# facebook/transform360

Measured on NVIDIA H100. Metric: Mpixels/s 8K equirect->cubemap bicubic (input-plane pixels consumed per second), higher is better.
Workload: dtype u8

## Files before the change

### include/transform360_b200.h

```cpp
#ifndef TRANSFORM360_B200_EXT_H
#define TRANSFORM360_B200_EXT_H

#include "Transform360/VideoFrameTransformHandler.h"

#ifdef __cplusplus
extern "C" {
#endif

typedef struct T360HostPlan T360HostPlan;

T360HostPlan* T360B200_hostPlanCreate(const FrameTransformContext* ctx, int inputWidth, int inputHeight,
                                      int outputWidth, int outputHeight);
#define T360_BORDER_WRAP 3
#define T360_BORDER_TRANSPARENT 5
T360HostPlan* T360B200_hostPlanCreateFromWarp(const FrameTransformContext* ctx, const float* map, int mapWidth, int mapHeight,
                                              int inputWidth, int inputHeight, int border);
void T360B200_hostPlanDestroy(T360HostPlan* plan);
int T360B200_hostPlanInfo(const T360HostPlan* plan, int info[6]);
const float* T360B200_hostPlanMap(const T360HostPlan* plan);
const int32_t* T360B200_hostPlanSamples(const T360HostPlan* plan);
int T360B200_hostPlanGather(T360HostPlan* plan, int info[10], const int32_t** jobs, const int32_t** records,
                            const uint32_t** compact);
int T360B200_hostPlanPoleCaps(T360HostPlan* plan, int info[4], const int32_t** capJobs, const uint32_t** capRecords,
                              const int32_t** launchJobs);
int T360B200_hostPlanDeviceLists(T360HostPlan* plan, int info[2], const int32_t** jobs, const uint32_t** records);
int T360B200_dealLanes(int interpolationAlg, int n, const int32_t* phases, int32_t* laneOf, int32_t* copyOf);
int T360B200_weightImage(int interpolationAlg, const uint8_t** image);
int T360B200_hostPlanBlurLists(T360HostPlan* const* plans, int numPlans, int width, int height, int layout[15],
                               const uint8_t** image);
int T360B200_hostPlanSegment(const T360HostPlan* plan, int i, int rect[4], int numTaps[2], const float** kx,
                             const float** ky);
int T360B200_remapTable(int interpolationAlg, const int16_t** table);

int T360B200_generateMapFromWarp(VideoFrameTransform* transform, const float* map, int mapWidth, int mapHeight, int inputWidth,
                                 int inputHeight, int border, int transformMatPlaneIndex);
int T360B200_remapFrameAsync(VideoFrameTransform* transform, int numPlanes, const float* const* deviceMaps, const int* mapPitches,
                             int border, const uint8_t* const* deviceInputs, uint8_t* const* deviceOutputs, const int* inputWidths,
                             const int* inputHeights, const int* inputPitches, const int* outputWidths, const int* outputHeights,
                             const int* outputPitches, void* cudaStream);

int T360B200_transformFramePlaneAsync(VideoFrameTransform* transform, const uint8_t* deviceInput,
                                      uint8_t* deviceOutput, int inputWidth, int inputHeight, int inputPitch,
                                      int outputWidth, int outputHeight, int outputPitch,
                                      int transformMatPlaneIndex, void* cudaStream);
int T360B200_transformFrameAsync(VideoFrameTransform* transform, int numPlanes, const uint8_t* const* deviceInputs,
                                 uint8_t* const* deviceOutputs, const int* inputWidths, const int* inputHeights,
                                 const int* inputPitches, const int* outputWidths, const int* outputHeights,
                                 const int* outputPitches, void* cudaStream);
int T360B200_lowPassPlaneAsync(VideoFrameTransform* transform, const uint8_t* deviceInput, uint8_t* deviceOutput,
                               int width, int height, int inputPitch, int outputPitch,
                               int transformMatPlaneIndex, void* cudaStream);
int T360B200_reconfigure(VideoFrameTransform* transform, const FrameTransformContext* ctx);
int T360B200_reconfigureAsync(VideoFrameTransform* transform, const FrameTransformContext* ctx);
int T360B200_reconfigureWait(VideoFrameTransform* transform, int block);
typedef struct T360View {
  float yaw, pitch, hfov, vfov;
} T360View;
int T360B200_transformFrameViewAsync(VideoFrameTransform* transform, const T360View* view, int numPlanes,
                                     const uint8_t* const* deviceInputs, uint8_t* const* deviceOutputs, const int* inputWidths,
                                     const int* inputHeights, const int* inputPitches, const int* outputWidths,
                                     const int* outputHeights, const int* outputPitches, void* cudaStream);
int T360B200_viewSamples(const FrameTransformContext* ctx, const T360View* view, int inputWidth, int inputHeight,
                         int outputWidth, int outputHeight, int32_t* samples);
typedef struct T360Orientation {
  float yaw, pitch, roll;
} T360Orientation;
int T360B200_transformFrameOrientedAsync(VideoFrameTransform* transform, const T360Orientation* orientation, int numPlanes,
                                         const uint8_t* const* deviceInputs, uint8_t* const* deviceOutputs,
                                         const int* inputWidths, const int* inputHeights, const int* inputPitches,
                                         const int* outputWidths, const int* outputHeights, const int* outputPitches,
                                         void* cudaStream);
int T360B200_orientedSamples(const FrameTransformContext* ctx, const T360Orientation* orientation, int inputWidth,
                             int inputHeight, int outputWidth, int outputHeight, int32_t* samples);
typedef struct T360Pose {
  float yaw, pitch, roll, hfov, vfov;
} T360Pose;
int T360B200_transformFramePoseAsync(VideoFrameTransform* transform, const T360Pose* pose, int numPlanes,
                                     const uint8_t* const* deviceInputs, uint8_t* const* deviceOutputs, const int* inputWidths,
                                     const int* inputHeights, const int* inputPitches, const int* outputWidths,
                                     const int* outputHeights, const int* outputPitches, void* cudaStream);
int T360B200_poseSamples(const FrameTransformContext* ctx, const T360Pose* pose, int inputWidth, int inputHeight,
                         int outputWidth, int outputHeight, int32_t* samples);
typedef struct T360Lens {
  float fx, fy, cx, cy;
  float k[4];
  float yaw, pitch, roll;
  float maxAngle;
} T360Lens;
typedef struct T360LensRig {
  int numLenses, calibWidth, calibHeight;
  T360Lens lens[2];
} T360LensRig;
int T360B200_lensMap(const FrameTransformContext* ctx, const T360LensRig* rig, const T360Orientation* orientation, int inputWidth,
                     int inputHeight, int outputWidth, int outputHeight, float* map);
int T360B200_transformFrameLensAsync(VideoFrameTransform* transform, const T360LensRig* rig, const T360Orientation* orientation,
                                     int numPlanes, const uint8_t* const* deviceInputs, uint8_t* const* deviceOutputs,
                                     const int* inputWidths, const int* inputHeights, const int* inputPitches,
                                     const int* outputWidths, const int* outputHeights, const int* outputPitches, void* cudaStream);
int T360B200_lensBlendMaps(const FrameTransformContext* ctx, const T360LensRig* rig, float seamWidth, const T360Orientation* orientation,
                           int inputWidth, int inputHeight, int outputWidth, int outputHeight, float* map0, float* map1, uint16_t* weight);
int T360B200_transformFrameLensBlendAsync(VideoFrameTransform* transform, const T360LensRig* rig, float seamWidth,
                                          const T360Orientation* orientation, int numPlanes, const uint8_t* const* deviceInputs,
                                          uint8_t* const* deviceOutputs, const int* inputWidths, const int* inputHeights,
                                          const int* inputPitches, const int* outputWidths, const int* outputHeights,
                                          const int* outputPitches, void* cudaStream);
int T360B200_rectilinearMap(const FrameTransformContext* ctx, const T360LensRig* rig, const T360Pose* pose, int inputWidth, int inputHeight,
                            int outputWidth, int outputHeight, float* map);
int T360B200_transformFrameRectilinearAsync(VideoFrameTransform* transform, const T360LensRig* rig, const T360Pose* pose, int numPlanes,
                                            const uint8_t* const* deviceInputs, uint8_t* const* deviceOutputs, const int* inputWidths,
                                            const int* inputHeights, const int* inputPitches, const int* outputWidths,
                                            const int* outputHeights, const int* outputPitches, void* cudaStream);
#define T360_CAMERA_PINHOLE 0
#define T360_CAMERA_EQUIDISTANT 1
#define T360_CAMERA_STEREOGRAPHIC 2
#define T360_CAMERA_PANNINI 3
typedef struct T360Camera {
  int model;
  float pannini;
} T360Camera;
int T360B200_cameraMap(const FrameTransformContext* ctx, const T360LensRig* rig, const T360Pose* pose, const T360Camera* camera,
                       int inputWidth, int inputHeight, int outputWidth, int outputHeight, float* map);
int T360B200_transformFrameCameraAsync(VideoFrameTransform* transform, const T360LensRig* rig, const T360Pose* pose, const T360Camera* camera,
                                       int numPlanes, const uint8_t* const* deviceInputs, uint8_t* const* deviceOutputs,
                                       const int* inputWidths, const int* inputHeights, const int* inputPitches, const int* outputWidths,
                                       const int* outputHeights, const int* outputPitches, void* cudaStream);
void T360B200_setPinHostPlanes(VideoFrameTransform* transform, int enable);
void T360B200_debugTrace(VideoFrameTransform* transform, int enable);
unsigned long long T360B200_debugTraceRead(VideoFrameTransform* transform, unsigned long long* out, unsigned long long maxWords);
int T360B200_synchronize(VideoFrameTransform* transform);
void* T360B200_stream(VideoFrameTransform* transform);

unsigned long long T360B200_kernelLaunchCount(void);
unsigned long long T360B200_planDeviceBytes(VideoFrameTransform* transform, int transformMatPlaneIndex);
int T360B200_planTileCounts(VideoFrameTransform* transform, int transformMatPlaneIndex, int counts[4]);
int T360B200_deviceCount(void);
const char* T360B200_version(void);

#ifdef __cplusplus
}
#endif
#endif
```

### transform360_b200/__init__.py

```python
from .handler import (BORDER_TRANSPARENT, BORDER_WRAP, CUBIC, LANCZOS4, LAYOUT_BARREL, LAYOUT_BARREL_SPLIT, LAYOUT_CUBEMAP_23_OFFCENTER,
                      LAYOUT_CUBEMAP_32, LAYOUT_EAC_32, LAYOUT_EQUIRECT, LAYOUT_FLAT_FIXED, LINEAR, NEAREST,
                      STEREO_FORMAT_GUESS, STEREO_FORMAT_LR, STEREO_FORMAT_MONO, STEREO_FORMAT_TB, T360_CAMERA_EQUIDISTANT, T360_CAMERA_PANNINI,
                      T360_CAMERA_PINHOLE, T360_CAMERA_STEREOGRAPHIC,
                      FrameTransformContext, HostPlan, T360Camera, T360Lens, T360LensRig, T360Orientation, T360Pose, T360View, VideoFrameTransform, device_count, kernel_launch_count,
                      camera_map, lens_blend_maps, lens_map, load, make_context, oriented_samples, pose_samples, rectilinear_map, remap_table,
                      square_pixel_vfov, view_samples, weight_image, deal_lanes)
```

### transform360_b200/csrc/gather_frame.cu

```cuda
#include "gather_common.cuh"

#include <cuda.h>

#include <algorithm>
#include <cstring>
#include <utility>

namespace t360 {

namespace {

template <class F, int... I>
__device__ __forceinline__ void staticForImpl(F&& f, std::integer_sequence<int, I...>) {
  (f(std::integral_constant<int, I>{}), ...);
}
template <int N, class F>
__device__ __forceinline__ void staticFor(F&& f) {
  staticForImpl(f, std::make_integer_sequence<int, N>{});
}

template <int IMM>
__device__ __forceinline__ uint32_t ldsWordImm(uint32_t addr) {
  uint32_t v;
  asm volatile("ld.shared.u32 %0, [%1+%2];" : "=r"(v) : "r"(addr), "n"(IMM));
  return v;
}
template <int IMM>
__device__ __forceinline__ uint4 ldsVecImm(uint32_t addr) {
  uint4 v;
  asm volatile("ld.shared.v4.u32 {%0, %1, %2, %3}, [%4+%5];" : "=r"(v.x), "=r"(v.y), "=r"(v.z), "=r"(v.w) : "r"(addr), "n"(IMM));
  return v;
}
template <int IMM>
__device__ __forceinline__ uint2 ldsVec2Imm(uint32_t addr) {
  uint2 v;
  asm volatile("ld.shared.v2.u32 {%0, %1}, [%2+%3];" : "=r"(v.x), "=r"(v.y) : "r"(addr), "n"(IMM));
  return v;
}

__device__ __forceinline__ uint32_t smemAddr(const void* p) { return (uint32_t)__cvta_generic_to_shared(p); }

__device__ __forceinline__ void mbarInit(uint64_t* bar, uint32_t arrivals) {
  asm volatile("mbarrier.init.shared::cta.b64 [%0], %1;" ::"r"(smemAddr(bar)), "r"(arrivals));
}
__device__ __forceinline__ void mbarExpectTx(uint64_t* bar, uint32_t bytes) {
  asm volatile("mbarrier.arrive.expect_tx.shared::cta.b64 _, [%0], %1;" ::"r"(smemAddr(bar)), "r"(bytes) : "memory");
}
__device__ __forceinline__ void mbarWait(uint64_t* bar, uint32_t parity) {
  asm volatile(
      "{\n\t.reg .pred p;\n\t"
      "WAIT_%=:\n\t"
      "mbarrier.try_wait.parity.shared::cta.b64 p, [%0], %1;\n\t"
      "@p bra DONE_%=;\n\t"
      "bra WAIT_%=;\n\t"
      "DONE_%=:\n\t}"
      ::"r"(smemAddr(bar)), "r"(parity) : "memory");
}
__device__ __forceinline__ void tmaLoadBox(void* dst, const CUtensorMap* map, int x, int y, uint64_t* bar) {
  asm volatile(
      "cp.async.bulk.tensor.2d.shared::cluster.global.mbarrier::complete_tx::bytes [%0], [%1, {%2, %3}], [%4];"
      ::"r"(smemAddr(dst)), "l"(reinterpret_cast<uint64_t>(map)), "r"(x), "r"(y), "r"(smemAddr(bar)) : "memory");
}
__device__ __forceinline__ void bulkCopyToShared(void* dst, const void* src, uint32_t bytes, uint64_t* bar) {
  asm volatile("cp.async.bulk.shared::cluster.global.mbarrier::complete_tx::bytes [%0], [%1], %2, [%3];"
               ::"r"(smemAddr(dst)), "l"(src), "r"(bytes), "r"(smemAddr(bar)) : "memory");
}
__device__ __forceinline__ void groupBarrier(int group) {
  asm volatile("bar.sync %0, %1;" ::"r"(group + 1), "n"(kGroupThreads) : "memory");
}

template <int K>
struct RowBytes {
  uint32_t b[K == 8 ? 2 : 1];
};

template <int K, int IMM>
__device__ __forceinline__ RowBytes<K> loadRow(uint32_t addr, int sh) {
  RowBytes<K> o;
  const uint32_t q0 = ldsWordImm<IMM>(addr), q1 = ldsWordImm<IMM + 4>(addr);
  o.b[0] = __funnelshift_r(q0, q1, sh);
  if constexpr (K == 8) o.b[1] = __funnelshift_r(q1, ldsWordImm<IMM + 8>(addr), sh);
  return o;
}

template <int K, int VS>
__device__ __forceinline__ int foldRows(const RowBytes<K> (&W)[K], uint32_t slotAddr) {
  int acc = 1 << 14;
  if constexpr (K == 2) {
    const uint2 w = ldsVec2Imm<0>(slotAddr);
    acc = dp2aLo(w.x, W[0].b[0], acc);
    acc = dp2aLo(w.y, W[1].b[0], acc);
  } else if constexpr (K == 4) {
    const uint4 wa = ldsVecImm<0>(slotAddr), wb = ldsVecImm<VS>(slotAddr);
    acc = dp2aLo(wa.x, W[0].b[0], acc); acc = dp2aHi(wa.y, W[0].b[0], acc);
    acc = dp2aLo(wa.z, W[1].b[0], acc); acc = dp2aHi(wa.w, W[1].b[0], acc);
    acc = dp2aLo(wb.x, W[2].b[0], acc); acc = dp2aHi(wb.y, W[2].b[0], acc);
    acc = dp2aLo(wb.z, W[3].b[0], acc); acc = dp2aHi(wb.w, W[3].b[0], acc);
  } else {
    staticFor<8>([&](auto R) {
      constexpr int r = decltype(R)::value;
      const uint4 wt = ldsVecImm<r * VS>(slotAddr);
      acc = dp2aLo(wt.x, W[r].b[0], acc); acc = dp2aHi(wt.y, W[r].b[0], acc);
      acc = dp2aLo(wt.z, W[r].b[1], acc); acc = dp2aHi(wt.w, W[r].b[1], acc);
    });
  }
  return acc;
}
template <int K>
__device__ __forceinline__ uint32_t slotOffset(uint32_t field) { return K == 2 ? field >> 1 : field; }

template <int VS>
__device__ __forceinline__ int foldRowsRotated(const RowBytes<8> (&W)[8], uint32_t wAddr, uint32_t field) {
  static_assert(VS == 16384, "one copy of the table");
  const uint32_t r = ((field >> 4) ^ threadIdx.x) & 7u;
  const uint32_t first = field ^ (r * (uint32_t)kDiagonalStep);
  const bool p0 = (r & 1u) != 0, p1 = (r & 2u) != 0, p2 = (r & 4u) != 0;
  RowBytes<8> A[8], B[8];
#pragma unroll
  for (int i = 0; i < 8; ++i)
#pragma unroll
    for (int h = 0; h < 2; ++h) A[i].b[h] = p0 ? W[i ^ 1].b[h] : W[i].b[h];
#pragma unroll
  for (int i = 0; i < 8; ++i)
#pragma unroll
    for (int h = 0; h < 2; ++h) B[i].b[h] = p1 ? A[i ^ 2].b[h] : A[i].b[h];
  int acc = 1 << 14;
  staticFor<8>([&](auto V) {
    constexpr int v = decltype(V)::value;
    const uint4 wt = ldsVecImm<0>(wAddr + (first ^ (uint32_t)(v * kDiagonalStep)));
    const uint32_t b0 = p2 ? B[v ^ 4].b[0] : B[v].b[0], b1 = p2 ? B[v ^ 4].b[1] : B[v].b[1];
    acc = dp2aLo(wt.x, b0, acc); acc = dp2aHi(wt.y, b0, acc);
    acc = dp2aLo(wt.z, b1, acc); acc = dp2aHi(wt.w, b1, acc);
  });
  return acc;
}
template <int K, int VS>
__device__ __forceinline__ int foldPixel(const RowBytes<K> (&W)[K], uint32_t wAddr, uint32_t field) {
  if constexpr (K == 8) return foldRowsRotated<VS>(W, wAddr, field);
  else return foldRows<K, VS>(W, wAddr + slotOffset<K>(field));
}
__device__ __forceinline__ int biasedToByte(int acc) { return min(max(acc >> 15, 0), 255); }


__device__ __forceinline__ uint32_t packBytes(int hi, int lo) {
  uint32_t r;
  asm("cvt.pack.sat.u8.s32.b32 %0, %1, %2, %3;" : "=r"(r) : "r"(hi), "r"(lo), "r"(0));
  return r;
}

template <int K, int PITCH, int VS, int ROWS, bool ZERO>
__device__ __forceinline__ void computeShareJob(uint8_t* dst, int dstPitch, uint32_t stageAddr, const uint4 (&rec)[ROWS / 8],
                                                uint32_t header, uint32_t wAddr) {
  static_assert(PITCH % 4 == 0 && (K == 4 || K == 8) && ROWS % 8 == 0, "");
  uint32_t base = stageAddr + (header & 0x7ffcu);
  const int sh = (int)(header << 3);
  RowBytes<K> W[K];
  staticFor<K>([&](auto R) { W[decltype(R)::value] = loadRow<K, decltype(R)::value * PITCH>(base, sh); });
  int accPrev = 0;
  staticFor<ROWS>([&](auto J) {
    constexpr int j = decltype(J)::value;
    const uint4& block = rec[j >> 3];
    const uint32_t word = ((j >> 1) & 3) == 0 ? block.x : (((j >> 1) & 3) == 1 ? block.y : (((j >> 1) & 3) == 2 ? block.z : block.w));
    const uint32_t r = (j & 1) ? word >> 16 : word;
    if constexpr (j > 0 && !ZERO) {
      const bool two = (r & 1u) != 0;
      const RowBytes<K> below = loadRow<K, (j - 1 + K) * PITCH>(base, sh);
      RowBytes<K> below2 = below;
      if (two) below2 = loadRow<K, (j + K) * PITCH>(base, sh);
#pragma unroll
      for (int q = 0; q + 2 < K; ++q)
#pragma unroll
        for (int i = 0; i < (K == 8 ? 2 : 1); ++i) W[q].b[i] = two ? W[q + 2].b[i] : W[q + 1].b[i];
#pragma unroll
      for (int i = 0; i < (K == 8 ? 2 : 1); ++i) W[K - 2].b[i] = two ? below.b[i] : W[K - 1].b[i];
      W[K - 1] = below2;
      if (two) base += PITCH;
    }
    if constexpr (j > 0 && ZERO) {
      const uint32_t d = r & 3u;
      RowBytes<K> below = W[K - 1], below2 = W[K - 1];
      if (d != 0) below = loadRow<K, K * PITCH>(base, sh);
      if (d == 2) below2 = loadRow<K, (K + 1) * PITCH>(base, sh);
#pragma unroll
      for (int q = 0; q + 2 < K; ++q)
#pragma unroll
        for (int i = 0; i < (K == 8 ? 2 : 1); ++i) W[q].b[i] = d == 0 ? W[q].b[i] : (d == 1 ? W[q + 1].b[i] : W[q + 2].b[i]);
#pragma unroll
      for (int i = 0; i < (K == 8 ? 2 : 1); ++i) {
        W[K - 2].b[i] = d == 0 ? W[K - 2].b[i] : (d == 1 ? W[K - 1].b[i] : below.b[i]);
        W[K - 1].b[i] = d == 0 ? W[K - 1].b[i] : (d == 1 ? below.b[i] : below2.b[i]);
      }
      base += d * PITCH;
    }
    const int acc = foldPixel<K, VS>(W, wAddr, r & kSlotFieldMask) >> 15;
    if constexpr (j & 1) {
      const uint32_t pair = packBytes(acc, accPrev);
      dst[(size_t)(j - 1) * dstPitch] = (uint8_t)pair;
      dst[(size_t)j * dstPitch] = (uint8_t)(pair >> 8);
    } else {
      accPrev = acc;
    }
  });
}

template <int K, int PITCH, int VS>
__device__ __forceinline__ void computeTileJob(const PlaneView& pv, uint32_t stageAddr, int outX, int outY, const uint4& rec,
                                               uint32_t wAddr, int warp) {
  static_assert(PITCH % 4 == 0, "");
  const int y0 = outY + warp * kTilePatchH;
  const int dstPitch = pv.dstPitch, dstW = pv.dstW, dstH = pv.dstH;
  uint8_t* const dstRow = pv.dst + (size_t)y0 * dstPitch + outX;
  const uint32_t words[4] = {rec.x, rec.y, rec.z, rec.w};
  staticFor<kRowsPerPatchStep>([&](auto J) {
    constexpr int j = decltype(J)::value;
    const uint32_t w = words[j];
    const int col = kTilePatchW * j + ((int)(w >> 16) & (kTilePatchW - 1)), row = (int)(w >> 19) & (kTilePatchH - 1);
    if (!(w & kRecordSkip) && outX + col < dstW && y0 + row < dstH) {
      const uint32_t rowAddr = stageAddr + (w & 0x7ffcu);
      const int sh = (int)(w << 3);
      RowBytes<K> W[K];
      staticFor<K>([&](auto R) { W[decltype(R)::value] = loadRow<K, decltype(R)::value * PITCH>(rowAddr, sh); });
      const int acc = foldPixel<K, VS>(W, wAddr, (w >> 17) & kSlotFieldMask);
      dstRow[(size_t)row * dstPitch + col] = (uint8_t)biasedToByte(acc);
    }
  });
}

template <int K, int PITCH, int VS>
__device__ __forceinline__ void computeCapJob(const PlaneView& pv, uint32_t stageAddr, uint32_t recAddr, int steps, uint32_t wAddr,
                                              int warp, int lane) {
  static_assert(PITCH % 4 == 0, "");
  for (int s = warp; s < steps; s += kGroupWarps) {
    const uint2 r = ldsVec2Imm<0>(recAddr + s * kCapStepBytes + lane * 8);
    if (r.x & kRecordSkip) continue;
    const uint32_t rowAddr = stageAddr + (r.x & 0x7ffcu);
    const int sh = (int)(r.x << 3);
    RowBytes<K> W[K];
    staticFor<K>([&](auto R) { W[decltype(R)::value] = loadRow<K, decltype(R)::value * PITCH>(rowAddr, sh); });
    const int acc = foldPixel<K, VS>(W, wAddr, (r.x >> 17) & kSlotFieldMask);
    pv.dst[(size_t)(r.y >> 16) * pv.dstPitch + (r.y & 0xffffu)] = (uint8_t)biasedToByte(acc);
  }
}

template <int K, int VS>
__device__ __forceinline__ void computeBorderJob(const PlaneView& pv, uint32_t recAddr, int n, const unsigned char* wsmem, int warp, int lane) {
  SrcView sv;
  sv.bytes = pv.src;
  sv.misalign = (int)(reinterpret_cast<uintptr_t>(pv.src) & 3);
  sv.words = reinterpret_cast<const uint32_t*>(pv.src - sv.misalign);
  sv.w = pv.srcW; sv.h = pv.srcH; sv.pitch = pv.srcPitch;
  for (int i = warp * 32 + lane; i < n; i += kGroupThreads) {
    const uint4 r = ldsVecImm<0>(recAddr + i * kBorderPixelBytes);
    const int v = gatherPixel<K, false, VS, weightDiagonal(K)>(sv, wsmem, (int)r.x, (int)r.y);
    pv.dst[(size_t)(r.z >> 16) * pv.dstPitch + (r.z & 0xffffu)] = (uint8_t)v;
  }
}

template <int K>
struct FrameTensorMaps {
  CUtensorMap map[kMaxFramePlanes][boxMaps(K)];
};

__device__ __forceinline__ void mbarArrive(uint64_t* bar) {
  asm volatile("mbarrier.arrive.shared::cta.b64 _, [%0];" ::"r"(smemAddr(bar)) : "memory");
}
__device__ __forceinline__ uint4 ldsVec(uint32_t addr) {
  uint4 v;
  asm volatile("ld.shared.v4.u32 {%0, %1, %2, %3}, [%4];" : "=r"(v.x), "=r"(v.y), "=r"(v.z), "=r"(v.w) : "r"(addr));
  return v;
}
__device__ __forceinline__ uint32_t ldsWord(uint32_t addr) {
  uint32_t v;
  asm volatile("ld.shared.u32 %0, [%1];" : "=r"(v) : "r"(addr));
  return v;
}

template <int K, int COPIES, int GROUPS>
struct FrameLayout {
  static constexpr int kStages = gatherStages(K);
  static constexpr int kWeights = weightImageBytes(K, COPIES);
  static constexpr int kStage = stageBytesOf(K), kRec = stageRecordBytes(K);
  static constexpr int kGroupBytes = kStages * (kStage + kRec);
  static constexpr int kPlanes = kWeights + GROUPS * kGroupBytes;
  static constexpr int kBars = kPlanes + 256;
  static constexpr int kTotal = kBars + GROUPS * kStages * 16 + 16;
  static_assert(kTotal <= 232448, "227 KB of shared memory per CTA");
  static_assert(sizeof(PlaneView) * kMaxFramePlanes <= 256, "");
  static_assert(kStage % 128 == 0 && kRec % 128 == 0 && kWeights % 128 == 0, "TMA / bulk-copy destinations");
};

template <int K, int COPIES, int GROUPS>
__global__ void __launch_bounds__(GROUPS * (kGroupWarps + 1) * 32, 1)
gatherFrameKernel(const __grid_constant__ FrameGatherParams p, StagedParams jobs, const __grid_constant__ FrameTensorMaps<K> maps) {
  using L = FrameLayout<K, COPIES, GROUPS>;
  constexpr int VS = weightVectorStride(K, COPIES), kStage = L::kStage, kRec = L::kRec, S = L::kStages;
  constexpr uint32_t kBox0 = stageBoxW(K, 0) * stageBoxH(K, 0), kBox1 = stageBoxW(K, 1) * stageBoxH(K, 1),
                     kBoxShare = stageBoxW(K, 2) * stageBoxH(K, 2);
  static_assert(kBox1 + 64 <= 2 * kStage && kBox0 + 64 <= kStage && kBoxShare + 64 <= kStage, "boxes must fit their stage buffers");
  static_assert(boxVariantRows(K, 0, kBoxVariants - 1) > 0 && boxVariantRows(K, 2, kBoxVariants - 1) > 0, "");
  extern __shared__ __align__(128) unsigned char smem[];
  unsigned char* wsmem = smem;
  PlaneView* planes = reinterpret_cast<PlaneView*>(smem + L::kPlanes);
  uint64_t* barBase = reinterpret_cast<uint64_t*>(smem + L::kBars);
  uint64_t* weightBar = barBase + GROUPS * 2 * S;
  const int warpId = threadIdx.x >> 5, lane = threadIdx.x & 31;
  constexpr int kProducerWarp = GROUPS * kGroupWarps;

  asm volatile("griddepcontrol.launch_dependents;" ::: "memory");
  if (threadIdx.x == 0) {
    for (int g = 0; g < GROUPS; ++g)
      for (int st = 0; st < S; ++st) {
        mbarInit(barBase + g * 2 * S + st, 1);
        mbarInit(barBase + g * 2 * S + S + st, kGroupWarps);
      }
    mbarInit(weightBar, 1);
    asm volatile("fence.mbarrier_init.release.cluster;" ::: "memory");
  }
  if (threadIdx.x < kMaxFramePlanes * (int)(sizeof(PlaneView) / 4))
    reinterpret_cast<uint32_t*>(planes)[threadIdx.x] = reinterpret_cast<const uint32_t*>(p.plane)[threadIdx.x];
  __syncthreads();

  if (warpId >= kProducerWarp) {
    const int g = warpId - kProducerWarp;
    if (g == 0 && lane == 0) {
      mbarExpectTx(weightBar, L::kWeights);
      constexpr int kChunk = L::kWeights / 4;
      for (int i = 0; i < 4; ++i)
        bulkCopyToShared(wsmem + i * kChunk, reinterpret_cast<const unsigned char*>(p.weightImage) + i * kChunk, kChunk, weightBar);
    }
    const int producer = blockIdx.x * GROUPS + g, dynamicBase = gridDim.x * GROUPS * 2;
    auto loadJob = [&](int i) {
      int4 h = make_int4(0, kJobExit << kJobKindShift, 0, 0);
      if (lane == 0 && i < jobs.numTiles) h = __ldg(reinterpret_cast<const int4*>(jobs.tiles) + i);
      return h;
    };
    int4 header = loadJob(producer * 2);
    int4 headerNext = loadJob(producer * 2 + 1);
    asm volatile("griddepcontrol.wait;" ::: "memory");
    int claimed = 0;
    if (lane == 0) claimed = atomicAdd(jobs.claimCounter, 1);
    unsigned char* groupBase = smem + L::kWeights + g * L::kGroupBytes;
    uint64_t* full = barBase + g * 2 * S;
    uint64_t* empty = full + S;
    uint32_t st = 0, phase = 0;
    auto advance = [&]() { if (++st == S) { st = 0; phase ^= 1; } };
    auto postEmptyJob = [&](int kind) {
      *reinterpret_cast<int4*>(groupBase + S * kStage + st * kRec) = make_int4(0, kind << kJobKindShift, 0, 0);
      mbarArrive(full + st);
    };
    for (;;) {
      int4 h;
      h.x = __shfl_sync(0xffffffffu, header.x, 0); h.y = __shfl_sync(0xffffffffu, header.y, 0);
      h.z = __shfl_sync(0xffffffffu, header.z, 0); h.w = __shfl_sync(0xffffffffu, header.w, 0);
      const int kind = (h.y >> kJobKindShift) & kJobKindMask;
      mbarWait(empty + st, phase ^ 1);
      const bool twoStages = kind == kJobClass1 || kind == kJobSeam;
      if (twoStages) {
        if (st == S - 1) {
          if (lane == 0) postEmptyJob(kJobNop);
          advance();
          mbarWait(empty + st, phase ^ 1);
        }
        mbarWait(empty + st + 1, phase ^ 1);
      }
      if (lane == 0) {
        unsigned char* rec = groupBase + S * kStage + st * kRec;
        *reinterpret_cast<int4*>(rec) = h;
        if (kind == kJobExit) {
          mbarArrive(full + st);
        } else {
          const int pl = h.y >> kJobPlaneShift;
          const uint32_t recBytes = (uint32_t)jobRecordBytes(K, kind, h.x);
          if (kind == kJobBorder) {
            mbarExpectTx(full + st, recBytes);
          } else {
            const int cls = boxClassOf(kind), variant = jobBoxVariant(h.z), boxX = jobBoxX(h.z), boxY = jobBoxY(h.z);
            const int width = (int)((unsigned)h.w >> kJobWidthShift);
            const uint32_t boxBytes = (uint32_t)((cls == 0 ? class0BoxW(width) : stageBoxW(K, cls)) * boxVariantRows(K, cls, variant));
            mbarExpectTx(full + st, (kind == kJobSeam ? 2 : 1) * boxBytes + recBytes);
            tmaLoadBox(groupBase + st * kStage, &maps.map[pl][boxMapIndex(K, cls, width, variant)], boxX, boxY, full + st);
            if (kind == kJobSeam)
              tmaLoadBox(groupBase + (st + 1) * kStage, &maps.map[pl][boxMapIndex(K, 0, 0, variant)], boxX - planes[pl].srcW, boxY, full + st);
          }
          bulkCopyToShared(rec + 128, planes[pl].records + ((unsigned)h.w & kJobRecordMask), recBytes, full + st);
        }
      }
      advance();
      if (twoStages) {
        if (lane == 0) postEmptyJob(kJobNop);
        advance();
      }
      __syncwarp();
      if (kind == kJobExit) break;
      header = headerNext;
      headerNext = loadJob(dynamicBase + __shfl_sync(0xffffffffu, claimed, 0));
      if (lane == 0) claimed = atomicAdd(jobs.claimCounter, 1);
    }
    if (lane == 0 && atomicAdd(jobs.claimCounter + 1, 1) == (int)(gridDim.x * GROUPS) - 1) {
      jobs.claimCounter[0] = 0;
      jobs.claimCounter[1] = 0;
      __threadfence();
    }
    return;
  }

  const int group = warpId / kGroupWarps, warp = warpId % kGroupWarps;
  unsigned char* groupBase = smem + L::kWeights + group * L::kGroupBytes;
  const uint32_t boxAddr = smemAddr(groupBase), recAddr = smemAddr(groupBase + S * kStage);
  uint64_t* full = barBase + group * 2 * S;
  uint64_t* empty = full + S;
  const uint32_t wAddr = smemAddr(wsmem);
  mbarWait(weightBar, 0);
  asm volatile("griddepcontrol.wait;" ::: "memory");
  auto now = []() { unsigned long long t; asm volatile("mov.u64 %0, %globaltimer;" : "=l"(t)); return t; };
  unsigned long long* trace = jobs.trace && warp == 0 && lane == 0 ? jobs.trace + (size_t)(blockIdx.x * GROUPS + group) * kTraceJobsPerGroup * 4 : nullptr;
  uint32_t traced = 0;
  for (uint32_t st = 0, phase = 0;;) {
    unsigned long long* const row = trace && traced < kTraceJobsPerGroup ? trace + traced * 4 : nullptr;
    if (row) row[0] = now();
    mbarWait(full + st, phase);
    if (row) row[1] = now();
    const uint32_t rec = recAddr + st * kRec;
    const uint4 h = ldsVec(rec);
    const int kind = ((int)h.y >> kJobKindShift) & kJobKindMask;
    if (kind == kJobExit) break;
    const int outX = (int)h.x & ~kJobQuadMask, outY = (int)h.y & kJobRowMask;
    const PlaneView& pv = planes[(int)h.y >> kJobPlaneShift];
    if (kind == kJobShare || kind == kJobShareStay) {
      if constexpr (K >= 4) {
        const uint32_t mine = rec + 128 + warp * shareWarpRecordBytes(K);
        uint4 r[shareRows(K) / 8];
#pragma unroll
        for (int b = 0; b < shareRows(K) / 8; ++b) r[b] = ldsVec(mine + b * 512 + lane * 16);
        const uint32_t header = ldsWord(mine + shareRows(K) / 8 * 512 + lane * 4);
        uint8_t* dst = pv.dst + (size_t)(outY + (warp >> 1) * shareRows(K)) * pv.dstPitch + (outX + (warp & 1) * 32 + (int)(header >> kRecordColumnShift));
        if (kind == kJobShare) computeShareJob<K, stageBoxW(K, 2), VS, shareRows(K), false>(dst, pv.dstPitch, boxAddr + st * kStage, r, header, wAddr);
        else computeShareJob<K, stageBoxW(K, 2), VS, shareRows(K), true>(dst, pv.dstPitch, boxAddr + st * kStage, r, header, wAddr);
      }
    } else if (kind == kJobClass0) {
      uint4 r;
      const int quad = ((int)h.x & kJobQuadMask) - 1;
      if (quad < 0) {
        r = ldsVec(rec + 128 + warp * 512 + lane * 16);
      } else {
        r = make_uint4(kRecordSkip, kRecordSkip, kRecordSkip, kRecordSkip);
        if ((warp >> 2) == (quad >> 1)) {
          const uint2 v = ldsVec2Imm<0>(rec + 128 + (warp & 3) * 256 + lane * 8);
          if (quad & 1) { r.z = v.x; r.w = v.y; } else { r.x = v.x; r.y = v.y; }
        }
      }
      const int width = (int)(h.w >> kJobWidthShift);
      staticFor<class0Widths(K)>([&](auto W) {
        constexpr int w = decltype(W)::value;
        if (width == w) computeTileJob<K, class0BoxW(w), VS>(pv, boxAddr + st * kStage, outX, outY, r, wAddr, warp);
      });
    } else if (kind == kJobClass1) {
      computeTileJob<K, stageBoxW(K, 1), VS>(pv, boxAddr + st * kStage, outX, outY, ldsVec(rec + 128 + warp * 512 + lane * 16), wAddr, warp);
    } else if (kind == kJobSeam) {
      {
        uint4* a = reinterpret_cast<uint4*>(groupBase + st * kStage);
        const uint4* b = reinterpret_cast<const uint4*>(groupBase + (st + 1) * kStage);
        for (int i = warp * 32 + lane; i < (int)(kBox0 / 16); i += kGroupThreads) {
          uint4 x = a[i];
          const uint4 y = b[i];
          x.x |= y.x; x.y |= y.y; x.z |= y.z; x.w |= y.w;
          a[i] = x;
        }
        asm volatile("fence.proxy.async.shared::cta;" ::: "memory");
      }
      groupBarrier(group);
      computeTileJob<K, stageBoxW(K, 0), VS>(pv, boxAddr + st * kStage, outX, outY, ldsVec(rec + 128 + warp * 512 + lane * 16), wAddr, warp);
    } else if (kind == kJobCap) {
      computeCapJob<K, stageBoxW(K, 0), VS>(pv, boxAddr + st * kStage, rec + 128, (int)h.x, wAddr, warp, lane);
    } else if (kind == kJobBorder) {
      computeBorderJob<K, VS>(pv, rec + 128, (int)h.x, wsmem, warp, lane);
    }
    __syncwarp();
    if (lane == 0) mbarArrive(empty + st);
    if (row) {
      row[2] = now(); row[3] = kind;
      ++traced;
    }
    if (++st == S) { st = 0; phase ^= 1; }
  }
}

template <int K, int COPIES, int GROUPS>
cudaError_t prepareFrameK(LaunchCfg& cfg) {
  static DeviceLaunchCfg cfgs;
  constexpr int threads = GROUPS * (kGroupWarps + 1) * 32, smemBytes = FrameLayout<K, COPIES, GROUPS>::kTotal;
  return prepare<gatherFrameKernel<K, COPIES, GROUPS>>(cfgs, threads, smemBytes, cfg);
}

template <int K, int COPIES, int GROUPS>
cudaError_t launchFrameK(const FrameGatherParams& p, const StagedParams& jobs, const void* tensorMaps, int numSMs,
                         cudaStream_t stream, bool programmatic) {
  FrameTensorMaps<K> maps;
  for (int i = 0; i < kMaxFramePlanes; ++i)
    std::memcpy(maps.map[i], static_cast<const CUtensorMap*>(tensorMaps) + (size_t)(i < p.numPlanes ? i : 0) * kMaxBoxMaps,
                sizeof(maps.map[i]));
  constexpr int threads = GROUPS * (kGroupWarps + 1) * 32, smemBytes = FrameLayout<K, COPIES, GROUPS>::kTotal;
  LaunchCfg cfg;
  cudaError_t err = prepareFrameK<K, COPIES, GROUPS>(cfg);
  if (err != cudaSuccess) return err;
  const int grid = std::min(numSMs * cfg.perSM, (jobs.numTiles + GROUPS * 2 - 1) / (GROUPS * 2));
  cudaLaunchConfig_t lc{};
  lc.gridDim = dim3(grid);
  lc.blockDim = dim3(threads);
  lc.dynamicSmemBytes = smemBytes;
  lc.stream = stream;
  cudaLaunchAttribute attr{};
  attr.id = cudaLaunchAttributeProgrammaticStreamSerialization;
  attr.val.programmaticStreamSerializationAllowed = 1;
  lc.attrs = &attr;
  lc.numAttrs = programmatic ? 1 : 0;
  err = cudaLaunchKernelEx(&lc, gatherFrameKernel<K, COPIES, GROUPS>, p, jobs, maps);
  gLaunches.fetch_add(1, std::memory_order_relaxed);
  return err;
}

}

cudaError_t prepareGatherFrame(int kernelSize) {
  LaunchCfg cfg;
  switch (kernelSize) {
    case 2: return prepareFrameK<2, weightCopies(2), gatherGroups(2)>(cfg);
    case 4: return prepareFrameK<4, weightCopies(4), gatherGroups(4)>(cfg);
    case 8: return prepareFrameK<8, weightCopies(8), gatherGroups(8)>(cfg);
    default: return cudaErrorInvalidValue;
  }
}

cudaError_t launchGatherFrame(const FrameGatherParams& p, const StagedParams& jobs, const void* tensorMaps, int numSMs,
                              cudaStream_t stream, bool programmatic) {
  if (jobs.numTiles <= 0) return cudaSuccess;
  if (p.numPlanes < 1 || p.numPlanes > kMaxFramePlanes) return cudaErrorInvalidValue;
  switch (p.kernelSize) {
    case 2: return launchFrameK<2, weightCopies(2), gatherGroups(2)>(p, jobs, tensorMaps, numSMs, stream, programmatic);
    case 4: return launchFrameK<4, weightCopies(4), gatherGroups(4)>(p, jobs, tensorMaps, numSMs, stream, programmatic);
    case 8: return launchFrameK<8, weightCopies(8), gatherGroups(8)>(p, jobs, tensorMaps, numSMs, stream, programmatic);
    default: return cudaErrorInvalidValue;
  }
}

}
```

### transform360_b200/csrc/kernels.cuh

```cuda
#pragma once

#include <cuda_runtime.h>

#include <cstdint>

#include "flat_view.h"
#include "oriented_view.h"

namespace t360 {

struct GatherParams {
  const uint8_t* src;
  int srcW, srcH, srcPitch;
  uint8_t* dst;
  int dstW, dstH, dstPitch;
  const int2* samples;
  int tilesPerRow;
  const int16_t* weights;
  int kernelSize;
  int transparent;
};

struct GatherJob {
  int outX, outY;
  int boxXY;
  int recordOffset;
};
constexpr int kBoxVariants = 3;
__host__ __device__ constexpr int jobBoxField(int boxX, int boxY, int variant) { return boxX | (boxY << 16) | variant; }
__host__ __device__ constexpr int jobBoxX(int boxXY) { return boxXY & 0xfff0; }
__host__ __device__ constexpr int jobBoxY(int boxXY) { return (int)((unsigned)boxXY >> 16); }
__host__ __device__ constexpr int jobBoxVariant(int boxXY) { return boxXY & 15; }
using StagedTile = GatherJob;
constexpr int kJobClass0 = 0, kJobClass1 = 1, kJobGeneral = 2, kJobShareStay = 3, kJobShare = 4, kJobNop = 5, kJobExit = 6, kJobSeam = 7,
              kJobCap = 8, kJobBorder = 9;
constexpr int kJobQuadMask = 7;
constexpr uint32_t kRecordSkip = 0x8000u;
constexpr int kJobKindShift = 24, kJobRowMask = (1 << kJobKindShift) - 1;
constexpr int kJobPlaneShift = 28, kJobKindMask = (1 << (kJobPlaneShift - kJobKindShift)) - 1;

constexpr int kGroupThreads = 256, kGroupWarps = kGroupThreads / 32;
__host__ __device__ constexpr int gatherGroups(int k) { return k == 8 ? 2 : 3; }
constexpr int kGatherTileW = 32, kFrameTileH = 32;
constexpr int kTilePatchW = 8, kTilePatchH = 4, kRowsPerPatchStep = 4;
constexpr int kShareW = 64;
__host__ __device__ constexpr int shareRows(int ) { return 8; }
__host__ __device__ constexpr int shareH(int k) { return 4 * shareRows(k); }
constexpr int kNumBoxClasses = 3;
__host__ __device__ constexpr int boxClassOf(int kind) { return (kind == kJobShare || kind == kJobShareStay) ? 2 : (kind == kJobClass1 ? 1 : 0); }
__host__ __device__ constexpr int stageBoxW(int , int cls) { return cls == 2 ? 192 : (cls == 0 ? 208 : 240); }
__host__ __device__ constexpr int stageBoxH(int k, int cls) {
  return k == 8 ? (cls == 2 ? 80 : (cls == 0 ? 72 : 128)) : (cls == 2 ? 72 : (cls == 0 ? 64 : 96));
}
__host__ __device__ constexpr int boxVariantRows(int k, int cls, int v) {
  return cls == 1 || v == 0 ? stageBoxH(k, cls) : (cls == 2 ? stageBoxH(k, cls) - 8 * v : stageBoxH(k, cls) - 8 - 8 * v);
}
__host__ __device__ constexpr int boxVariantFor(int k, int cls, int rows) {
  int v = 0;
  while (v + 1 < kBoxVariants && cls != 1 && boxVariantRows(k, cls, v + 1) >= rows) ++v;
  return v;
}
constexpr int kClass0Widths = 4, kJobWidthShift = 28, kJobRecordMask = (1 << kJobWidthShift) - 1;
__host__ __device__ constexpr int class0BoxW(int w) { return w == 0 ? 208 : (w == 1 ? 144 : (w == 2 ? 112 : 80)); }
__host__ __device__ constexpr int class0Widths(int k) { return k == 8 ? 1 : kClass0Widths; }
__host__ __device__ constexpr int class0WidthFor(int k, int cols) {
  int w = 0;
  while (w + 1 < class0Widths(k) && class0BoxW(w + 1) >= cols) ++w;
  return w;
}
__host__ __device__ constexpr int boxMaps(int k) { return class0Widths(k) * kBoxVariants + 1 + kBoxVariants; }
constexpr int kMaxBoxMaps = kClass0Widths * kBoxVariants + 1 + kBoxVariants;
__host__ __device__ constexpr int boxMapIndex(int k, int cls, int width, int variant) {
  return cls == 0 ? width * kBoxVariants + variant : (cls == 1 ? class0Widths(k) * kBoxVariants : class0Widths(k) * kBoxVariants + 1 + variant);
}
__host__ __device__ constexpr int boxMapClass(int k, int i) {
  return i < class0Widths(k) * kBoxVariants ? 0 : (i == class0Widths(k) * kBoxVariants ? 1 : 2);
}
__host__ __device__ constexpr int boxMapW(int k, int i) { return boxMapClass(k, i) == 0 ? class0BoxW(i / kBoxVariants) : stageBoxW(k, boxMapClass(k, i)); }
__host__ __device__ constexpr int boxMapRows(int k, int i) {
  return boxMapClass(k, i) == 0 ? boxVariantRows(k, 0, i % kBoxVariants)
         : boxMapClass(k, i) == 1 ? stageBoxH(k, 1)
                                  : boxVariantRows(k, 2, i - class0Widths(k) * kBoxVariants - 1);
}

__host__ __device__ constexpr int gatherStages(int ) { return 2; }
__host__ __device__ constexpr int stageBytesOf(int k) {
  const int a = stageBoxW(k, 2) * stageBoxH(k, 2), b = stageBoxW(k, 0) * stageBoxH(k, 0);
  return ((a > b ? a : b) + 64 + 127) & ~127;
}

__host__ __device__ constexpr int weightSlotOf(int k, int phase) {
  (void)k;
  return (phase & ~31) | ((phase & 1) << 4) | ((phase & 31) >> 1);
}
__host__ __device__ constexpr int weightCopies(int k) { return k == 4 ? 2 : 1; }
__host__ __device__ constexpr int weightVectorStride(int k, int copies) { return (k == 2 ? 8192 : 16384) * copies; }
__host__ __device__ constexpr int weightImageBytes(int k, int copies) { return k == 2 ? 8192 * copies : (k * k / 8) * 16384 * copies; }
__host__ __device__ constexpr int weightSlotInCopy(int slot, int copy) { return copy ? ((slot & ~7) | ((slot + copy) & 7)) : slot; }
__host__ __device__ constexpr int weightSlotField(int k, int phase, int copy) {
  return (weightSlotInCopy(weightSlotOf(k, phase), copy) << 4) | (copy << 14);
}
constexpr int kSlotFieldMask = 0x7FF0;
constexpr int kDiagonalStep = 0x4010;
__host__ __device__ constexpr bool weightDiagonal(int k) { return k == 8; }
__host__ __device__ constexpr int weightVectorOffset(int k, int copies, int slotFieldValue, int vector) {
  return weightDiagonal(k) ? (slotFieldValue ^ (vector * kDiagonalStep)) : slotFieldValue + vector * weightVectorStride(k, copies);
}
__host__ __device__ constexpr int weightBankGroups(int k) { return k == 2 ? 16 : 8; }
__host__ __device__ constexpr int weightLanesPerPass(int k) { return k == 2 ? 16 : 8; }

__host__ __device__ constexpr int shareWarpRecordBytes(int k) { return shareRows(k) / 8 * 32 * 16 + 32 * 4; }
__host__ __device__ constexpr int shareJobRecordBytes(int k) { return kGroupWarps * shareWarpRecordBytes(k); }
constexpr int kTileJobRecordBytes = kGroupWarps * 32 * 16;
constexpr int kQuadJobRecordBytes = kGroupWarps / 2 * 32 * 8;
__host__ __device__ constexpr int tileJobRecordBytes(int outXField) { return (outXField & kJobQuadMask) ? kQuadJobRecordBytes : kTileJobRecordBytes; }
__host__ __device__ constexpr int stageRecordBytes(int k) {
  return 128 + (shareJobRecordBytes(k) > kTileJobRecordBytes ? shareJobRecordBytes(k) : kTileJobRecordBytes);
}
constexpr int kCapStepBytes = 32 * 8, kBorderPixelBytes = 16;
__host__ __device__ constexpr int capJobMaxSteps(int k) { return (stageRecordBytes(k) - 128) / kCapStepBytes; }
__host__ __device__ constexpr int borderJobMaxPixels(int k) { return (stageRecordBytes(k) - 128) / kBorderPixelBytes; }
__host__ __device__ constexpr int jobRecordBytes(int k, int kind, int outXField) {
  return kind == kJobShare || kind == kJobShareStay ? shareJobRecordBytes(k)
         : kind == kJobCap                          ? outXField * kCapStepBytes
         : kind == kJobBorder                       ? outXField * kBorderPixelBytes
                                                    : tileJobRecordBytes(outXField);
}
constexpr int kRecordColumnShift = 27;

constexpr int kMaxFramePlanes = 3;
struct PlaneView {
  const uint8_t* src;
  uint8_t* dst;
  const uint4* records;
  int srcW, srcH, srcPitch;
  int dstW, dstH, dstPitch;
};
struct FrameGatherParams {
  PlaneView plane[kMaxFramePlanes];
  const uint4* weightImage;
  int kernelSize, numPlanes;
};

__host__ __device__ constexpr int gatherThreads(int k) { return k == 8 ? 512 : 256; }
__host__ __device__ constexpr int gatherTileH(int k) { return gatherThreads(k) / 32 * 4; }

struct StagedParams {
  const GatherJob* tiles;
  int numTiles;
  int* claimCounter;
  unsigned long long* trace;
};
constexpr int kTraceJobsPerGroup = 64;

struct BlurJob {
  int x0, y0, w, h;
  int kxOffset, kxCount, kyOffset, kyCount;
};

struct BlurParams {
  const uint8_t* src;
  uint8_t* dst;
  int width, height, srcPitch, dstPitch;
  const BlurJob* jobs;
  int numJobs;
  const float* taps;
  int tileSmemBytes;
};

struct StripJob {
  int x0, y0, w, h;
  int kxOffset, kxChunks, kxCount, kyOffset;
  int edge;
};

struct StripParams {
  const uint8_t* src;
  uint8_t* dst;
  int width, height, srcPitch, dstPitch;
  const StripJob* jobs;
  int numJobs;
  const float* taps;
};

struct AreaParams {
  const uint8_t* src;
  uint8_t* dst;
  int srcW, srcH, srcPitch, dstW, dstH, dstPitch;
  int cellW, cellH;
  const int2* xTaps;
  const int* xFirst;
  const int2* yTaps;
  const int* yFirst;
  const int2* xLinear;
  const int2* yLinear;
  int xMax;
};
cudaError_t launchAreaResize(const AreaParams& p, cudaStream_t stream);

struct FrameStripParams {
  struct Plane {
    const uint8_t* src;
    uint8_t* dst;
    int width, height, srcPitch, dstPitch;
  } plane[kMaxFramePlanes];
  int numPlanes;
  const StripJob* jobs;
  int numJobs;
  const float* taps;
};
constexpr int kStripPlaneShift = 8;
cudaError_t launchBlurFrameStrips(const FrameStripParams& p, int hy, cudaStream_t stream);

constexpr int kStripLanePx = 8, kStripW = 32 * kStripLanePx, kStripMaxHy = 3;

constexpr int kBlurTileW = 64, kBlurTileH = 32;
constexpr int kBlurMaxSmem = 96 * 1024;

cudaError_t launchGather(const GatherParams& p, int numSMs, cudaStream_t stream);
cudaError_t launchGatherFrame(const FrameGatherParams& p, const StagedParams& jobs, const void* tensorMaps, int numSMs,
                              cudaStream_t stream, bool programmatic = true);
cudaError_t prepareGatherFrame(int kernelSize);
cudaError_t launchBlur(const BlurParams& p, cudaStream_t stream);
cudaError_t launchBlurDirect(const BlurParams& p, cudaStream_t stream);
unsigned long long kernelLaunchCount();
void countKernelLaunches(long long n);

enum class PerFrameSource { kView, kSphere, kMap, kLens, kLensBlend, kRectilinear };
struct PerFramePlane {
  const uint8_t* src;
  uint8_t* dst;
  int srcPitch, dstPitch;
  SphereGeometry geometry;
  const float* colTable;
  const float* rowTable;
  int tilesX, firstTile;
  const float2* map;
  int mapPitch;
};
struct PerFrameGatherParams {
  PerFramePlane plane[kMaxFramePlanes];
  int numPlanes;
  FlatView view;
  Rotation rotation;
  LensRigModel rig;
  RectilinearCamera camera;
  float seamScale;
  bool transparent;
  bool lens;
  const int16_t* weights;
  int kernelSize;
};
constexpr int kViewRowsPerThread = 8;
__host__ __device__ constexpr int viewTileRows(int k) { return gatherThreads(k) / 32 * kViewRowsPerThread; }
cudaError_t launchPerFrameGather(PerFrameGatherParams p, PerFrameSource source, int numSMs, cudaStream_t stream);

inline int blurTileSmem(int w, int h, int nkx, int nky) {
  const int hx = nkx / 2, hy = nky / 2;
  const int rows = h + 2 * hy;
  const int srcStride = (w + 2 * hx + 3) & ~3;
  return rows * srcStride + rows * w * 4;
}

}
```

### transform360_b200/csrc/video_frame_transform.cpp

```cpp
#include <cuda.h>
#include <cuda_runtime.h>

#include <algorithm>
#include <chrono>
#include <climits>
#include <cmath>
#include <condition_variable>
#include <cstdarg>
#include <cstdio>
#include <cstdlib>
#include <cstring>
#include <map>
#include <memory>
#include <mutex>
#include <new>
#include <shared_mutex>
#include <stdexcept>
#include <string>
#include <string_view>
#include <thread>
#include <vector>

#include "host_plan.h"
#include "gather_plan.h"
#include "kernels.cuh"
#include "lowpass_jobs.h"
#include "transform360_b200.h"

#define T360_API extern "C" __attribute__((visibility("default")))

namespace {

using t360::BlurJob;
using t360::GatherJob;
using t360::HostPlan;
using t360::StripJob;

struct CudaFail {
  cudaError_t err;
  const char* what;
};

#define CU(call)                                       \
  do {                                                 \
    cudaError_t e__ = (call);                          \
    if (e__ != cudaSuccess) throw CudaFail{e__, #call}; \
  } while (0)

template <class Body>
bool guarded(std::string_view what, Body&& body) {
  const int n = static_cast<int>(what.size());
  try {
    return body();
  } catch (const CudaFail& f) {
    std::printf("%.*s. Error: CUDA %s (%s) in %s\n", n, what.data(), cudaGetErrorName(f.err), cudaGetErrorString(f.err), f.what);
    cudaGetLastError();
  } catch (const std::exception& ex) {
    std::printf("%.*s. Error: %s\n", n, what.data(), ex.what());
  }
  return false;
}

template <typename T>
struct DeviceBuffer {
  T* ptr = nullptr;
  size_t count = 0;
  DeviceBuffer() = default;
  DeviceBuffer(const DeviceBuffer&) = delete;
  DeviceBuffer& operator=(const DeviceBuffer&) = delete;
  DeviceBuffer(DeviceBuffer&& o) noexcept : ptr(o.ptr), count(o.count) { o.ptr = nullptr; o.count = 0; }
  DeviceBuffer& operator=(DeviceBuffer&& o) noexcept {
    if (this != &o) { release(); ptr = o.ptr; count = o.count; o.ptr = nullptr; o.count = 0; }
    return *this;
  }
  ~DeviceBuffer() { release(); }
  void release() {
    if (ptr) cudaFree(ptr);
    ptr = nullptr;
    count = 0;
  }
  void reserve(size_t n) {
    if (n <= count) return;
    release();
    CU(cudaMalloc(reinterpret_cast<void**>(&ptr), n * sizeof(T)));
    count = n;
  }
  size_t bytes() const { return count * sizeof(T); }
};

struct DevicePlan {
  int inW = 0, inH = 0, outW = 0, outH = 0, mapW = 0, mapH = 0;
  int kernelSize = 0;
  bool transparent = false, lowPass = false;
  bool warp = false;
  int stereoFormat = STEREO_FORMAT_MONO;
  DeviceBuffer<int2> samples;
  DeviceBuffer<uint32_t> records;
  int tilesPerRow = 0;
  DeviceBuffer<GatherJob> gatherJobs;
  std::vector<GatherJob> hostJobs;
  std::vector<int> jobNeedRows;
  std::vector<t360::JobRect> jobRects;
  int numJobs = 0, numStaged = 0, numBorder = 0;
  struct BlurSet {
    t360::BlurLists lists;
    t360::BlurLayout layout;
    DeviceBuffer<uint8_t> image;
    bool needsClear = false;
  };
  BlurSet blur;
  std::vector<t360::LowPassSegment> segments;
  std::vector<float> planTaps;
  mutable std::map<std::pair<int, int>, BlurSet> otherBlurs;
  struct Resize {
    int cellW = 0, cellH = 0, xMax = 0;
    DeviceBuffer<int2> xTaps, yTaps, xLinear, yLinear;
    DeviceBuffer<int> xFirst, yFirst;
  };
  bool resizeNeeded = false;
  mutable std::map<std::pair<int, int>, Resize> resizes;
  DeviceBuffer<float> sphereTables;
  size_t deviceBytes() const {
    return samples.bytes() + records.bytes() + gatherJobs.bytes() + blur.image.bytes();
  }
};

bool mergeable(const DevicePlan* const* plans, const t360::BlurLists* const* lists, const bool* clear, int numPlanes, const int* inW,
               const int* inH) {
  if (numPlanes < 2) return false;
  for (int p = 0; p < numPlanes; ++p) {
    const DevicePlan& d = *plans[p];
    if (d.transparent || inW[p] != d.inW || inH[p] != d.inH || clear[p] || !lists[p]->tiles.empty() || !lists[p]->direct.empty())
      return false;
  }
  return true;
}

struct HostIndexPlan {
  HostPlan host;
  t360::GatherPlan gather;
};
void gatherOnHost(HostIndexPlan& p) {
  if (p.host.kernelSize > 0) t360::buildGatherPlan(p.host, p.host.kernelSize >= 2 && !p.host.transparentBorder, p.gather);
}
bool planOnHost(const FrameTransformContext& ctx, int inW, int inH, int outW, int outH, HostIndexPlan& p) {
  if (!t360::buildHostPlan(ctx, inW, inH, outW, outH, p.host)) return false;
  gatherOnHost(p);
  return true;
}
bool planWarpOnHost(const FrameTransformContext& ctx, const float* map, int mapW, int mapH, int inW, int inH, int border, HostIndexPlan& p) {
  if (!t360::buildWarpHostPlan(ctx, map, mapW, mapH, inW, inH, border, p.host)) return false;
  gatherOnHost(p);
  return true;
}

void* driverEntry(const char* name) {
  void* p = nullptr;
  cudaDriverEntryPointQueryResult q{};
  if (cudaGetDriverEntryPoint(name, &p, cudaEnableDefault, &q) != cudaSuccess || q != cudaDriverEntryPointSuccess) {
    cudaGetLastError();
    p = nullptr;
  }
  return p;
}

constexpr std::chrono::milliseconds kSettleInterval{250};

using EncodeTiledFn = CUresult (*)(CUtensorMap*, CUtensorMapDataType, cuuint32_t, void*, const cuuint64_t*, const cuuint64_t*,
                                   const cuuint32_t*, const cuuint32_t*, CUtensorMapInterleave, CUtensorMapSwizzle,
                                   CUtensorMapL2promotion, CUtensorMapFloatOOBfill);

EncodeTiledFn tensorMapEncoder() {
  static const EncodeTiledFn fn = reinterpret_cast<EncodeTiledFn>(driverEntry("cuTensorMapEncodeTiled"));
  return fn;
}

bool encodePlaneMap(CUtensorMap* map, const uint8_t* base, int w, int h, int pitch, int k, int index) {
  EncodeTiledFn enc = tensorMapEncoder();
  if (!enc) return false;
  if ((reinterpret_cast<uintptr_t>(base) & 15) || (pitch & 15)) return false;
  const cuuint64_t dims[2] = {static_cast<cuuint64_t>(w), static_cast<cuuint64_t>(h)};
  const cuuint64_t strides[1] = {static_cast<cuuint64_t>(pitch)};
  const cuuint32_t box[2] = {static_cast<cuuint32_t>(t360::boxMapW(k, index)), static_cast<cuuint32_t>(t360::boxMapRows(k, index))};
  const cuuint32_t elem[2] = {1, 1};
  return enc(map, CU_TENSOR_MAP_DATA_TYPE_UINT8, 2, const_cast<uint8_t*>(base), dims, strides, box, elem,
             CU_TENSOR_MAP_INTERLEAVE_NONE, CU_TENSOR_MAP_SWIZZLE_NONE, CU_TENSOR_MAP_L2_PROMOTION_L2_128B,
             CU_TENSOR_MAP_FLOAT_OOB_FILL_NONE) == CUDA_SUCCESS;
}

constexpr int kPlaneLanes = 3;
static_assert(kPlaneLanes == t360::kMaxFramePlanes, "the frame kernel takes one PlaneView per lane");
struct PlaneMaps {
  const uint8_t* base = nullptr;
  int w = 0, h = 0, pitch = 0, k = 0;
  CUtensorMap maps[t360::kMaxBoxMaps];
};
struct PlaneLane {
  static constexpr int kMapCache = 32;
  PlaneMaps mapCache[kMapCache];
  int mapCacheNext = 0;
  cudaStream_t main = nullptr;
  cudaEvent_t done = nullptr;
  DeviceBuffer<uint8_t> blurred;
  DeviceBuffer<uint8_t> scaled;
  DeviceBuffer<int> claimCounter;
};

struct PlaneTarget {
  uint8_t* dst = nullptr;
  int dstPitch = 0, dstW = 0, dstH = 0;
  uint8_t* out = nullptr;
  int outPitch = 0, outW = 0, outH = 0;
  const DevicePlan::Resize* resize = nullptr;
};

struct GatherWork {
  const DevicePlan* plan = nullptr;
  t360::PlaneView view{};
  bool staged = false;
  CUtensorMap maps[t360::kMaxBoxMaps];
  PlaneTarget target;
};

struct FrameLists {
  unsigned long long generation = ~0ull;
  DeviceBuffer<GatherJob> gatherJobs;
  int numGatherJobs = 0;
  DeviceBuffer<uint8_t> blurImage;
  t360::BlurLayout blurLayout;
};
struct FrameListRefs {
  const GatherJob* gatherJobs;
  int numGatherJobs;
  const uint8_t* blurImage;
  t360::BlurLayout blurLayout;
};

struct WavePlan {
  struct Rect { int x, y, w, h; };
  int chunks = 0;
  const void* plan = nullptr;
  unsigned long long generation = ~0ull;
  std::vector<int> chunkRowEnd, waveStart;
  DeviceBuffer<GatherJob> jobs;
  std::vector<std::vector<Rect>> rects;
};

struct PlaneGraph {
  const void* plan; unsigned long long generation; const void* in; const void* out; int inPitch, outPitch;
  const void* stagingIn; const void* stagingOut;
  int inW, inH, outW, outH;
  int kernels;
  cudaGraphExec_t exec; unsigned long long lastUse;
};

struct ViewBlurCache {
  std::vector<long long> key;
  bool merged = false;
  std::vector<uint8_t> jobs;
  std::vector<int> tapCodes;
  t360::BlurLayout layout[2];
  bool clear[2] = {false, false};
};

struct UploadRing {
  static constexpr int kEntries = 3;
  struct Entry {
    uint8_t* host = nullptr;
    uint8_t* device = nullptr;
    size_t capacity = 0;
    cudaEvent_t released = nullptr;
    bool inFlight = false;
  };
  Entry entries[kEntries];
  int last = -1;
  std::vector<uint8_t> lastContent;
};

struct StreamSlot {
  PlaneLane lanes[kPlaneLanes];
  DeviceBuffer<int> frameClaim;
  cudaEvent_t fork = nullptr;
  UploadRing viewJobs, viewTaps;
  ViewBlurCache viewBlur;
  UploadRing sphereTables;
  std::vector<uint8_t> sphereBytes;
  size_t sphereAt[kPlaneLanes] = {SIZE_MAX, SIZE_MAX, SIZE_MAX};
  FrameTransformContext sphereCtx{};
  std::vector<int> sphereSizes;
};

int scratchPlane(DeviceBuffer<uint8_t>& buf, int w, int h) {
  constexpr int kPitchAlign = 256;
  const int pitch = (w + kPitchAlign - 1) / kPitchAlign * kPitchAlign;
  buf.reserve(static_cast<size_t>(pitch) * h + 64);
  return pitch;
}

struct FramePlanes {
  int numPlanes = 0;
  const uint8_t* in[kPlaneLanes];
  uint8_t* out[kPlaneLanes];
  int inW[kPlaneLanes], inH[kPlaneLanes], inPitch[kPlaneLanes], outW[kPlaneLanes], outH[kPlaneLanes], outPitch[kPlaneLanes];
};

bool describeFrame(const char* what, int numPlanes, const uint8_t* const* dIn, uint8_t* const* dOut, const int* inW, const int* inH,
                   const int* inPitch, const int* outW, const int* outH, const int* outPitch, FramePlanes& f) {
  if (!dIn || !dOut || !inW || !inH || !inPitch || !outW || !outH || !outPitch) {
    std::printf("%s. Error: a NULL argument\n", what);
    return false;
  }
  if (numPlanes < 1 || numPlanes > kPlaneLanes) {
    std::printf("%s. Error: %d planes (1..%d supported)\n", what, numPlanes, kPlaneLanes);
    return false;
  }
  f.numPlanes = numPlanes;
  for (int p = 0; p < numPlanes; ++p) {
    if (!dIn[p] || !dOut[p] || inW[p] <= 0 || inH[p] <= 0 || outW[p] <= 0 || outH[p] <= 0 || inPitch[p] < inW[p] || outPitch[p] < outW[p]) {
      std::printf("%s. Error: invalid description of plane %d\n", what, p);
      return false;
    }
    f.in[p] = dIn[p]; f.out[p] = dOut[p];
    f.inW[p] = inW[p]; f.inH[p] = inH[p]; f.inPitch[p] = inPitch[p];
    f.outW[p] = outW[p]; f.outH[p] = outH[p]; f.outPitch[p] = outPitch[p];
  }
  return true;
}

void setPose(FrameTransformContext& ctx, const T360Pose& pose) {
  ctx.fixed_yaw = pose.yaw;
  ctx.fixed_pitch = pose.pitch;
  ctx.fixed_roll = pose.roll;
  ctx.fixed_hfov = pose.hfov;
  ctx.fixed_vfov = pose.vfov;
}

std::string formatted(const char* fmt, ...) __attribute__((format(printf, 1, 2)));
std::string formatted(const char* fmt, ...) {
  char buf[320];
  va_list args;
  va_start(args, fmt);
  std::vsnprintf(buf, sizeof(buf), fmt, args);
  va_end(args);
  return buf;
}

std::string withFields(FrameTransformContext& ctx, const T360Pose& pose) {
  if (!std::isfinite(pose.yaw) || !std::isfinite(pose.pitch) || !std::isfinite(pose.roll) || !std::isfinite(pose.hfov) ||
      !std::isfinite(pose.vfov))
    return formatted("the pose (yaw %g, pitch %g, roll %g, hfov %g, vfov %g) is not finite", pose.yaw, pose.pitch, pose.roll, pose.hfov,
                     pose.vfov);
  if (ctx.output_layout < 0 || ctx.output_layout >= LAYOUT_N) return formatted("output_layout %d is not a layout", static_cast<int>(ctx.output_layout));
  setPose(ctx, pose);
  return {};
}
std::string withFields(FrameTransformContext& ctx, const T360View& view) {
  if (!std::isfinite(view.yaw) || !std::isfinite(view.pitch) || !std::isfinite(view.hfov) || !std::isfinite(view.vfov))
    return formatted("the view (yaw %g, pitch %g, hfov %g, vfov %g) is not finite", view.yaw, view.pitch, view.hfov, view.vfov);
  if (ctx.output_layout != LAYOUT_FLAT_FIXED)
    return formatted("per-frame views need output_layout FLAT_FIXED (%d), the transform has %d", static_cast<int>(LAYOUT_FLAT_FIXED),
                     static_cast<int>(ctx.output_layout));
  setPose(ctx, T360Pose{view.yaw, view.pitch, ctx.fixed_roll, view.hfov, view.vfov});
  return {};
}
std::string withFields(FrameTransformContext& ctx, const T360Orientation& o) {
  if (!std::isfinite(o.yaw) || !std::isfinite(o.pitch) || !std::isfinite(o.roll))
    return formatted("the orientation (yaw %g, pitch %g, roll %g) is not finite", o.yaw, o.pitch, o.roll);
  if (!t360::orientedLayouts(ctx))
    return formatted("per-frame orientations need output_layout CUBEMAP_32, CUBEMAP_23_OFFCENTER, EAC_32 or EQUIRECT and input_layout "
                     "EQUIRECT or CUBEMAP_32, the transform has %d -> %d%s", static_cast<int>(ctx.input_layout),
                     static_cast<int>(ctx.output_layout),
                     ctx.output_layout == LAYOUT_FLAT_FIXED ? " (FLAT_FIXED views: T360B200_transformFrameViewAsync)" : "");
  setPose(ctx, T360Pose{o.yaw, o.pitch, o.roll, ctx.fixed_hfov, ctx.fixed_vfov});
// ... 433 lines not shown
      int dInPitch = inPitch, dOutPitch = outPitch;
      if (!inOnDevice) {
        pinIfRecurring(in, static_cast<size_t>(inPitch) * (inH - 1) + inW);
        dInPitch = scratchPlane(stagingIn_, inW, inH);
        CU(cudaMemcpy2DAsync(stagingIn_.ptr, dInPitch, in, inPitch, inW, inH, cudaMemcpyHostToDevice, stream_));
        dIn = stagingIn_.ptr;
      }
      if (!outOnDevice) {
        pinIfRecurring(out, static_cast<size_t>(outPitch) * (outH - 1) + outW);
        dOutPitch = scratchPlane(stagingOut_, outW, outH);
        dOut = stagingOut_.ptr;
        if (plan->transparent && !planIndex)
          CU(cudaMemcpy2DAsync(dOut, dOutPitch, out, outPitch, outW, outH, cudaMemcpyHostToDevice, stream_));
      }
      if (!enqueue(*plan, planIndex != 0, dIn, dOut, inW, inH, dInPitch, outW, outH, dOutPitch, stream_, imagePlaneIndex,
                   slotFor(stream_).lanes[0]))
        return false;
      if (!outOnDevice)
        CU(cudaMemcpy2DAsync(out, outPitch, dOut, dOutPitch, outW, outH, cudaMemcpyDeviceToHost, stream_));
      CU(cudaStreamSynchronize(stream_));
      return true;
    });
  }

  bool pipelineEligible(const DevicePlan& plan, int inW, int inH, int outW, int outH) const {
    return plan.numJobs > 0 && !plan.transparent && !plan.lowPass && inW == plan.inW && inH == plan.inH &&
           outW == plan.mapW && outH == plan.mapH && static_cast<long long>(inW) * inH >= pipelineMinBytes_ && inH >= 64;
  }

  WavePlan& wavePlanFor(const DevicePlan& plan, int planIndex, int chunks) {
    WavePlan& w = wavePlans_[planIndex ? 1 : 0];
    if (w.plan == &plan && w.chunks == chunks && w.generation == planGeneration_) return w;
    w.chunks = chunks;
    w.plan = &plan;
    w.generation = planGeneration_;
    const int rowsPer = ((plan.inH + chunks - 1) / chunks + 7) & ~7;
    w.chunkRowEnd.assign(chunks, plan.inH);
    for (int c = 0; c < chunks; ++c) w.chunkRowEnd[c] = std::min(plan.inH, (c + 1) * rowsPer);
    auto waveOf = [&](int needRows) {
      int c = 0;
      while (c + 1 < chunks && w.chunkRowEnd[c] < needRows) ++c;
      return c;
    };
    std::vector<std::vector<GatherJob>> byWave(chunks);
    const int bands = (plan.mapH + 31) / 32;
    std::vector<int> complete(bands, 0);
    for (size_t i = 0; i < plan.hostJobs.size(); ++i) {
      const int c = waveOf(plan.jobNeedRows[i]);
      byWave[c].push_back(plan.hostJobs[i]);
      const t360::JobRect& r = plan.jobRects[i];
      for (int band = r.y0 / 32; band <= (r.y1 - 1) / 32; ++band) complete[band] = std::max(complete[band], c);
    }
    std::vector<GatherJob> all;
    w.waveStart.assign(chunks + 1, 0);
    for (int c = 0; c < chunks; ++c) {
      w.waveStart[c] = static_cast<int>(all.size());
      all.insert(all.end(), byWave[c].begin(), byWave[c].end());
    }
    w.waveStart[chunks] = static_cast<int>(all.size());
    w.jobs.reserve(all.size());
    CU(cudaMemcpy(w.jobs.ptr, all.data(), all.size() * sizeof(GatherJob), cudaMemcpyHostToDevice));
    w.rects.assign(chunks, {});
    for (int band = 0; band < bands;) {
      const int c = complete[band];
      int end = band + 1;
      while (end < bands && complete[end] == c) ++end;
      w.rects[c].push_back(WavePlan::Rect{0, band * 32, plan.mapW, std::min(plan.mapH, end * 32) - band * 32});
      band = end;
    }
    return w;
  }

  PlaneGraph* findPlaneGraph(const DevicePlan& plan, const uint8_t* in, const uint8_t* out, int inW, int inH, int inPitch, int outW, int outH,
                             int outPitch) {
    PlaneGraph* g = nullptr;
    for (size_t i = 0; i < planeGraphs_.size();) {
      PlaneGraph& c = planeGraphs_[i];
      if (c.stagingIn != stagingIn_.ptr || c.stagingOut != stagingOut_.ptr || c.generation != planGeneration_) {
        cudaGraphExecDestroy(c.exec);
        planeGraphs_.erase(planeGraphs_.begin() + static_cast<long>(i));
        continue;
      }
      if (c.plan == &plan && c.in == in && c.out == out && c.inPitch == inPitch && c.outPitch == outPitch && c.inW == inW && c.inH == inH &&
          c.outW == outW && c.outH == outH)
        g = &c;
      ++i;
    }
    return g;
  }

  bool replayPlaneGraph(PlaneGraph& g) {
    g.lastUse = ++graphClock_;
    CU(cudaGraphLaunch(g.exec, stream_));
    t360::countKernelLaunches(g.kernels);
    CU(cudaStreamSynchronize(stream_));
    return true;
  }

  bool transformHostPlanePipelined(const DevicePlan& plan, uint8_t* in, uint8_t* out, int inW, int inH, int inPitch, int outW, int outH,
                                   int outPitch, int planIndex, int imagePlaneIndex) {
    const long long bytes = static_cast<long long>(inW) * inH;
    const int chunks = static_cast<int>(std::min<long long>(8, std::max<long long>(2, bytes / (3ll << 20))));
    WavePlan& w = wavePlanFor(plan, planIndex, chunks);
    if (!copyIn_) {
      CU(cudaStreamCreateWithFlags(&copyIn_, cudaStreamNonBlocking));
      CU(cudaStreamCreateWithFlags(&copyOut_, cudaStreamNonBlocking));
      for (cudaEvent_t* e : {&graphFork_, &graphJoinIn_, &graphJoinOut_}) CU(cudaEventCreateWithFlags(e, cudaEventDisableTiming));
    }
    while (static_cast<int>(chunkIn_.size()) < chunks) {
      cudaEvent_t a = nullptr, b = nullptr;
      CU(cudaEventCreateWithFlags(&a, cudaEventDisableTiming));
      chunkIn_.push_back(a);
      CU(cudaEventCreateWithFlags(&b, cudaEventDisableTiming));
      waveDone_.push_back(b);
    }
    pinIfRecurring(in, static_cast<size_t>(inPitch) * (inH - 1) + inW);
    pinIfRecurring(out, static_cast<size_t>(outPitch) * (outH - 1) + outW);
    const int dInPitch = scratchPlane(stagingIn_, inW, inH), dOutPitch = scratchPlane(stagingOut_, outW, outH);
    PlaneLane& hostLane = slotFor(stream_).lanes[0];
    GatherWork work;
    if (!prepareGather(plan, planIndex != 0, stagingIn_.ptr, stagingOut_.ptr, inW, inH, dInPitch, outW, outH, dOutPitch, stream_,
                       imagePlaneIndex, hostLane, work))
      return false;
    if (!work.staged) {
      CU(cudaMemcpy2DAsync(stagingIn_.ptr, dInPitch, in, inPitch, inW, inH, cudaMemcpyHostToDevice, stream_));
      gatherPlane(work, hostLane, stream_);
      CU(cudaMemcpy2DAsync(out, outPitch, stagingOut_.ptr, dOutPitch, outW, outH, cudaMemcpyDeviceToHost, stream_));
      CU(cudaStreamSynchronize(stream_));
      return true;
    }
    armScheduler(hostLane.claimCounter, stream_);
    CU(t360::prepareGatherFrame(plan.kernelSize));
    auto issue = [&](bool forkJoin) {
      if (forkJoin) {
        CU(cudaEventRecord(graphFork_, stream_));
        CU(cudaStreamWaitEvent(copyIn_, graphFork_, 0));
        CU(cudaStreamWaitEvent(copyOut_, graphFork_, 0));
      }
      t360::FrameGatherParams fp{};
      fp.plane[0] = work.view;
      fp.weightImage = reinterpret_cast<const uint4*>(weightImages_[plan.kernelSize].ptr);
      fp.kernelSize = plan.kernelSize;
      fp.numPlanes = 1;
      for (int c = 0; c < chunks; ++c) {
        const int r0 = c ? w.chunkRowEnd[c - 1] : 0, r1 = w.chunkRowEnd[c];
        if (r1 > r0)
          CU(cudaMemcpy2DAsync(stagingIn_.ptr + static_cast<size_t>(r0) * dInPitch, dInPitch, in + static_cast<size_t>(r0) * inPitch, inPitch, inW,
                               r1 - r0, cudaMemcpyHostToDevice, copyIn_));
        CU(cudaEventRecord(chunkIn_[c], copyIn_));
        CU(cudaStreamWaitEvent(stream_, chunkIn_[c], 0));
        const int n = w.waveStart[c + 1] - w.waveStart[c];
        if (n > 0) {
          t360::StagedParams jobs{w.jobs.ptr + w.waveStart[c], n, hostLane.claimCounter.ptr, nullptr};
          CU(t360::launchGatherFrame(fp, jobs, work.maps, numSMs_, stream_, false));
        }
        if (!w.rects[c].empty()) {
          CU(cudaEventRecord(waveDone_[c], stream_));
          CU(cudaStreamWaitEvent(copyOut_, waveDone_[c], 0));
          for (const WavePlan::Rect& r : w.rects[c])
            CU(cudaMemcpy2DAsync(out + static_cast<size_t>(r.y) * outPitch + r.x, outPitch,
                                 stagingOut_.ptr + static_cast<size_t>(r.y) * dOutPitch + r.x, dOutPitch, r.w, r.h, cudaMemcpyDeviceToHost, copyOut_));
        }
      }
      if (forkJoin) {
        CU(cudaEventRecord(graphJoinIn_, copyIn_));
        CU(cudaEventRecord(graphJoinOut_, copyOut_));
        CU(cudaStreamWaitEvent(stream_, graphJoinIn_, 0));
        CU(cudaStreamWaitEvent(stream_, graphJoinOut_, 0));
      }
    };
    if (memoryTypeOf(in) == cudaMemoryTypeHost && memoryTypeOf(out) == cudaMemoryTypeHost) {
      PlaneGraph* g = findPlaneGraph(plan, in, out, inW, inH, inPitch, outW, outH, outPitch);
      if (!g) {
        if (planeGraphs_.size() >= 24) {
          auto oldest = std::min_element(planeGraphs_.begin(), planeGraphs_.end(), [](const PlaneGraph& a, const PlaneGraph& b) { return a.lastUse < b.lastUse; });
          cudaGraphExecDestroy(oldest->exec);
          planeGraphs_.erase(oldest);
        }
        CU(cudaStreamSynchronize(stream_));
        cudaGraph_t graph = nullptr;
        CU(cudaStreamBeginCapture(stream_, cudaStreamCaptureModeThreadLocal));
        try {
          issue(true);
        } catch (...) {
          cudaStreamEndCapture(stream_, &graph);
          if (graph) cudaGraphDestroy(graph);
          throw;
        }
        CU(cudaStreamEndCapture(stream_, &graph));
        cudaGraphExec_t exec = nullptr;
        const cudaError_t e = cudaGraphInstantiate(&exec, graph, 0);
        cudaGraphDestroy(graph);
        if (e != cudaSuccess) throw CudaFail{e, "cudaGraphInstantiate"};
        int kernels = 0;
        for (int c = 0; c < chunks; ++c) kernels += w.waveStart[c + 1] > w.waveStart[c];
        planeGraphs_.push_back(PlaneGraph{&plan, planGeneration_, in, out, inPitch, outPitch, stagingIn_.ptr, stagingOut_.ptr, inW, inH, outW, outH,
                                          kernels, exec, 0});
        g = &planeGraphs_.back();
        t360::countKernelLaunches(-kernels);
      }
      return replayPlaneGraph(*g);
    }
    issue(false);
    CU(cudaStreamSynchronize(stream_));
    CU(cudaStreamSynchronize(copyOut_));
    return true;
  }

  bool transformDevice(const uint8_t* dIn, uint8_t* dOut, int inW, int inH, int inPitch, int outW, int outH,
                       int outPitch, int planIndex, cudaStream_t stream) {
    return guarded("Could not transform the plane " + std::to_string(planIndex), [&] {
      std::shared_lock<std::shared_mutex> config = lockPlanned("Could not transform the plane");
      if (!config.owns_lock()) return false;
      const DeviceRestore restoreDevice = ensureDevice();
      const DevicePlan* plan = findPlan(planIndex, planIndex);
      if (!plan) return false;
      cudaStream_t s = stream ? stream : stream_;
      return enqueue(*plan, planIndex != 0, dIn, dOut, inW, inH, inPitch, outW, outH, outPitch, s, planIndex, slotFor(s).lanes[0]);
    });
  }

  bool transformFrameDevice(const FramePlanes& f, cudaStream_t stream) {
    const int numPlanes = f.numPlanes;
    return guarded("Could not transform the frame", [&] {
      std::shared_lock<std::shared_mutex> config(configMu_);
      while (perFrameOnly_) {
        if (planesOfPlannedSize(f))
          return perFrameLocked("Could not transform the frame while its plan is pending", ctx_, f, stream);
        config.unlock();
        if (reconfigureWait(true) < 0) {
          std::printf("Could not transform the frame. Error: the background planner failed on the current context\n");
          return false;
        }
        config.lock();
      }
      const DeviceRestore restoreDevice = ensureDevice();
      cudaStream_t s = stream ? stream : stream_;
      StreamSlot& slot = slotFor(s);
      PlaneLane* lanes_ = slot.lanes;
      cudaEvent_t frameFork_ = slot.fork;
      const DevicePlan* plans[kPlaneLanes];
      bool sideWork = false;
      for (int p = 0; p < numPlanes; ++p) {
        if (!(plans[p] = findPlan(p ? 1 : 0, p))) return false;
        if (p) sideWork = sideWork || plans[p]->lowPass || plans[p]->transparent;
      }
      const t360::BlurLists* lists[kPlaneLanes];
      bool clear[kPlaneLanes], lowPass = true;
      for (int p = 0; p < numPlanes; ++p) {
        lists[p] = &plans[p]->blur.lists;
        clear[p] = plans[p]->blur.needsClear;
        lowPass = lowPass && plans[p]->lowPass;
      }
      const bool mergedBlur = lowPass && mergeable(plans, lists, clear, numPlanes, f.inW, f.inH);
      if (mergedBlur) {
        blurFrame(plans, f, lanes_, s);
        sideWork = false;
      }
      const bool fork = numPlanes > 1 && sideWork;
      if (fork) CU(cudaEventRecord(frameFork_, s));
      GatherWork work[kPlaneLanes];
      bool allStaged = true;
      for (int p = numPlanes - 1; p >= 0; --p) {
        cudaStream_t ps = (p && fork) ? lanes_[p].main : s;
        if (p && fork) CU(cudaStreamWaitEvent(ps, frameFork_, 0));
        if (!prepareGather(*plans[p], p > 0, f.in[p], f.out[p], f.inW[p], f.inH[p], f.inPitch[p], f.outW[p], f.outH[p], f.outPitch[p], ps, p,
                           lanes_[p], work[p], mergedBlur))
          return false;
        allStaged = allStaged && work[p].staged;
      }
      if (allStaged && numPlanes > 1) {
        if (fork)
          for (int p = 1; p < numPlanes; ++p) {
            CU(cudaEventRecord(lanes_[p].done, lanes_[p].main));
            CU(cudaStreamWaitEvent(s, lanes_[p].done, 0));
          }
        gatherFrame(work, numPlanes, s, slot);
        for (int p = 0; p < numPlanes; ++p) finishTarget(work[p].target, s);
        return true;
      }
      if (numPlanes > 1 && !fork) CU(cudaEventRecord(frameFork_, s));
      for (int p = numPlanes - 1; p >= 0; --p) {
        cudaStream_t ps = p ? lanes_[p].main : s;
        if (p && !fork) CU(cudaStreamWaitEvent(ps, frameFork_, 0));
        if (work[p].plan->kernelSize) {
          gatherPlane(work[p], lanes_[p], ps);
          finishTarget(work[p].target, ps);
        }
        if (p) CU(cudaEventRecord(lanes_[p].done, ps));
      }
      for (int p = 1; p < numPlanes; ++p) CU(cudaStreamWaitEvent(s, lanes_[p].done, 0));
      return true;
    });
  }

  bool lowPassDevice(const uint8_t* dIn, uint8_t* dOut, int w, int h, int inPitch, int outPitch, int planIndex,
                     cudaStream_t stream) {
    return guarded("Could not filter plane " + std::to_string(planIndex), [&] {
      std::shared_lock<std::shared_mutex> config = lockPlanned("Could not filter the plane");
      if (!config.owns_lock()) return false;
      const DeviceRestore restoreDevice = ensureDevice();
      const DevicePlan* plan = findPlan(planIndex, planIndex);
      if (!plan) return false;
      if (!plan->lowPass) {
        std::printf("Could not filter plane %d. Error: plan has no low-pass stage\n", planIndex);
        return false;
      }
// ... 288 lines not shown
    return buf.ptr;
  }

  DevicePlan upload(HostIndexPlan& p, const FrameTransformContext& ctx) {
    const HostPlan& h = p.host;
    DevicePlan d;
    d.inW = h.inW; d.inH = h.inH; d.outW = h.outW; d.outH = h.outH; d.mapW = h.mapW; d.mapH = h.mapH;
    d.kernelSize = h.kernelSize;
    d.transparent = h.transparentBorder;
    d.warp = h.warp;
    d.stereoFormat = ctx.input_stereo_format;
    if (d.kernelSize > 0) {
      deviceWeights(ctx.interpolation_alg);
      t360::GatherPlan& g = p.gather;
      d.tilesPerRow = g.tilesPerRow;
      d.samples.reserve(g.records.size());
      CU(cudaMemcpy(d.samples.ptr, g.records.data(), g.records.size() * sizeof(int2), cudaMemcpyHostToDevice));
      d.numStaged = g.totalStaged();
      d.numBorder = g.numBorder;
      d.numJobs = static_cast<int>(g.launchJobs.size());
      d.hostJobs = t360::deviceJobs(g);
      if (!d.hostJobs.empty()) {
        d.gatherJobs.reserve(d.hostJobs.size());
        CU(cudaMemcpy(d.gatherJobs.ptr, d.hostJobs.data(), d.hostJobs.size() * sizeof(GatherJob), cudaMemcpyHostToDevice));
      }
      if (!g.compact.empty() || !g.capRecords.empty()) {
        const std::vector<uint32_t> records = t360::deviceRecords(g, d.kernelSize);
        d.records.reserve(records.size());
        CU(cudaMemcpy(d.records.ptr, records.data(), records.size() * sizeof(uint32_t), cudaMemcpyHostToDevice));
      }
      d.jobNeedRows = std::move(g.launchNeedRows);
      d.jobRects = std::move(g.launchRects);
    }
    d.lowPass = ctx.enable_low_pass_filter != 0;
    if (d.lowPass) {
      d.segments = h.segments;
      d.planTaps = h.taps;
      buildBlurSet(d.segments, d.planTaps, h.inW, h.inH, d.stereoFormat, d.blur);
    }
    d.resizeNeeded = h.resize.needed;
    if (d.resizeNeeded) resizeFor(d, d.outW, d.outH);
    if (d.kernelSize > 0 && !d.warp && ctx.output_layout != LAYOUT_FLAT_FIXED) {
      const std::vector<float> t = t360::buildSphereTables(t360::sphereGeometry(ctx, h.mapW, h.mapH, h.inW, h.inH, h.kernelSize));
      if (!t.empty()) {
        d.sphereTables.reserve(t.size());
        CU(cudaMemcpy(d.sphereTables.ptr, t.data(), t.size() * sizeof(float), cudaMemcpyHostToDevice));
      }
    }
    return d;
  }

  const DevicePlan::Resize& resizeFor(const DevicePlan& plan, int outW, int outH) {
    std::lock_guard<std::mutex> lock(lazyMu_);
    auto it = plan.resizes.find({outW, outH});
    if (it != plan.resizes.end()) return it->second;
    t360::AreaResizePlan r;
    t360::buildAreaResize(plan.mapW, plan.mapH, outW, outH, r);
    DevicePlan::Resize& d = plan.resizes[{outW, outH}];
    auto upload2 = [](const std::vector<int2>& v, DeviceBuffer<int2>& buf) {
      buf.reserve(std::max<size_t>(v.size(), 1));
      if (!v.empty()) CU(cudaMemcpy(buf.ptr, v.data(), v.size() * sizeof(int2), cudaMemcpyHostToDevice));
    };
    if (r.enlarge) {
      d.cellW = d.cellH = -1;
      d.xMax = r.lx.dmax;
      auto pack = [](const t360::AreaLinearAxis& a) {
        std::vector<int2> v(a.ofs.size());
        for (size_t i = 0; i < a.ofs.size(); ++i)
          v[i] = int2{a.ofs[i], static_cast<int>(static_cast<uint16_t>(a.coef[2 * i]) | (static_cast<uint32_t>(static_cast<uint16_t>(a.coef[2 * i + 1])) << 16))};
        return v;
      };
      upload2(pack(r.lx), d.xLinear);
      upload2(pack(r.ly), d.yLinear);
    } else if (r.cellW > 0) {
      d.cellW = r.cellW; d.cellH = r.cellH;
    } else {
      auto uploadAxis = [&](const t360::AreaAxis& a, DeviceBuffer<int2>& taps, DeviceBuffer<int>& first) {
        std::vector<int2> packed(a.taps.size());
        for (size_t i = 0; i < a.taps.size(); ++i) {
          int bits;
          std::memcpy(&bits, &a.taps[i].alpha, sizeof(bits));
          packed[i] = int2{a.taps[i].src, bits};
        }
        upload2(packed, taps);
        first.reserve(a.first.size());
        CU(cudaMemcpy(first.ptr, a.first.data(), a.first.size() * sizeof(int), cudaMemcpyHostToDevice));
      };
      uploadAxis(r.x, d.xTaps, d.xFirst);
      uploadAxis(r.y, d.yTaps, d.yFirst);
    }
    return d;
  }

  void buildBlurSet(const std::vector<t360::LowPassSegment>& segments, const std::vector<float>& planTaps, int planeW, int planeH,
                    int stereoFormat, DevicePlan::BlurSet& d) {
    t360::buildBlurLists(segments, planTaps, planeW, planeH, stereoFormat, d.lists, &d.needsClear);
    std::vector<uint8_t> image;
    d.layout = t360::packBlurLists(d.lists, image, image);
    if (image.empty()) return;
    d.image.reserve(image.size());
    CU(cudaMemcpy(d.image.ptr, image.data(), image.size(), cudaMemcpyHostToDevice));
  }

  const DevicePlan::BlurSet& blurFor(const DevicePlan& plan, int w, int h) {
    if (w == plan.inW && h == plan.inH) return plan.blur;
    std::lock_guard<std::mutex> lock(lazyMu_);
    auto it = plan.otherBlurs.find({w, h});
    if (it != plan.otherBlurs.end()) return it->second;
    DevicePlan::BlurSet& set = plan.otherBlurs[{w, h}];
    buildBlurSet(plan.segments, plan.planTaps, w, h, plan.stereoFormat, set);
    return set;
  }

  void launchLowPass(const t360::BlurLayout& l, bool clear, const uint8_t* jobs, const uint8_t* taps, t360::FrameStripParams fp, int numPlanes,
                     cudaStream_t s) {
    const t360::FrameStripParams::Plane& a = fp.plane[0];
    if (clear)
      for (int p = 0; p < numPlanes; ++p) CU(cudaMemset2DAsync(fp.plane[p].dst, fp.plane[p].dstPitch, 0, fp.plane[p].width, fp.plane[p].height, s));
    fp.numPlanes = numPlanes;
    fp.taps = reinterpret_cast<const float*>(taps + l.tapAt);
    for (int c = 0; c < t360::kStripMaxHy; ++c) {
      if (!l.numStrips[c]) continue;
      fp.jobs = reinterpret_cast<const StripJob*>(jobs + l.stripAt[c]);
      fp.numJobs = l.numStrips[c];
      CU(t360::launchBlurFrameStrips(fp, c + 1, s));
    }
    t360::BlurParams bp{a.src, a.dst, a.width, a.height, a.srcPitch, a.dstPitch, reinterpret_cast<const BlurJob*>(jobs + l.tileAt), l.numTiles,
                        fp.taps, l.tileSmem};
    if (bp.numJobs) CU(t360::launchBlur(bp, s));
    if (l.numDirect) {
      bp.jobs = reinterpret_cast<const BlurJob*>(jobs + l.directAt);
      bp.numJobs = l.numDirect;
      CU(t360::launchBlurDirect(bp, s));
    }
  }

  void runLowPass(const DevicePlan& plan, const uint8_t* dIn, uint8_t* dOut, int w, int h, int inPitch, int outPitch,
                  cudaStream_t s) {
    const DevicePlan::BlurSet& b = blurFor(plan, w, h);
    t360::FrameStripParams fp{};
    fp.plane[0] = {dIn, dOut, w, h, inPitch, outPitch};
    launchLowPass(b.layout, b.needsClear, b.image.ptr, b.image.ptr, fp, 1, s);
  }

  static bool planeMaps(PlaneLane& lane, const uint8_t* src, int w, int h, int pitch, int k,
                        CUtensorMap (&out)[t360::kMaxBoxMaps]) {
    for (const PlaneMaps& e : lane.mapCache)
      if (e.base == src && e.w == w && e.h == h && e.pitch == pitch && e.k == k) {
        std::memcpy(out, e.maps, sizeof(e.maps));
        return true;
      }
    PlaneMaps fresh;
    for (int m = 0; m < t360::boxMaps(k); ++m)
      if (!encodePlaneMap(&fresh.maps[m], src, w, h, pitch, k, m)) return false;
    fresh.base = src; fresh.w = w; fresh.h = h; fresh.pitch = pitch; fresh.k = k;
    lane.mapCache[lane.mapCacheNext] = fresh;
    lane.mapCacheNext = (lane.mapCacheNext + 1) % PlaneLane::kMapCache;
    std::memcpy(out, fresh.maps, sizeof(fresh.maps));
    return true;
  }

  bool enqueue(const DevicePlan& plan, bool chroma, const uint8_t* dIn, uint8_t* dOut, int inW, int inH, int inPitch, int outW,
               int outH, int outPitch, cudaStream_t s, int imagePlaneIndex, PlaneLane& lane) {
    GatherWork w;
    if (!prepareGather(plan, chroma, dIn, dOut, inW, inH, inPitch, outW, outH, outPitch, s, imagePlaneIndex, lane, w)) return false;
    if (plan.kernelSize == 0) return true;
    gatherPlane(w, lane, s);
    finishTarget(w.target, s);
    return true;
  }

  bool prepareGather(const DevicePlan& plan, bool chroma, const uint8_t* dIn, uint8_t* dOut, int inW, int inH, int inPitch, int outW,
                     int outH, int outPitch, cudaStream_t s, int imagePlaneIndex, PlaneLane& lane, GatherWork& w, bool blurDone = false) {
    w.plan = &plan;
    if (plan.kernelSize == 0) {
      std::printf("Could not find interpolation algorithm for plane %d", imagePlaneIndex);
      return true;
    }
    const PlaneTarget& t = w.target = renderTarget(&plan, chroma, plan.transparent, dOut, outPitch, outW, outH, &lane.scaled, s);
    const uint8_t* src = dIn;
    int srcPitch = inPitch;
    if (plan.lowPass) {
      const int bp = scratchPlane(lane.blurred, inW, inH);
      if (!blurDone) runLowPass(plan, dIn, lane.blurred.ptr, inW, inH, inPitch, bp, s);
      src = lane.blurred.ptr;
      srcPitch = bp;
    }
    w.view = t360::PlaneView{src, t.dst, reinterpret_cast<const uint4*>(plan.records.ptr), inW, inH, srcPitch, t.dstW, t.dstH, t.dstPitch};
    w.staged = plan.numJobs > 0 && !plan.transparent && inW == plan.inW && inH == plan.inH;
    if (w.staged) w.staged = planeMaps(lane, src, inW, inH, srcPitch, plan.kernelSize, w.maps);
    return true;
  }

  static void armScheduler(DeviceBuffer<int>& counter, cudaStream_t s) {
    if (counter.ptr) return;
    counter.reserve(2);
    CU(cudaMemsetAsync(counter.ptr, 0, 2 * sizeof(int), s));
  }

  void gatherPlane(const GatherWork& w, PlaneLane& lane, cudaStream_t s) {
    const DevicePlan& plan = *w.plan;
    if (w.staged) {
      armScheduler(lane.claimCounter, s);
      t360::FrameGatherParams fp{};
      fp.plane[0] = w.view;
      fp.weightImage = reinterpret_cast<const uint4*>(weightImages_[plan.kernelSize].ptr);
      fp.kernelSize = plan.kernelSize;
      fp.numPlanes = 1;
      t360::StagedParams jobs{plan.gatherJobs.ptr, plan.numJobs, lane.claimCounter.ptr, nullptr};
      CU(t360::launchGatherFrame(fp, jobs, w.maps, numSMs_, s));
    } else {
      const t360::PlaneView& v = w.view;
      t360::GatherParams gp{v.src, v.srcW, v.srcH, v.srcPitch, v.dst, v.dstW, v.dstH, v.dstPitch, plan.samples.ptr, plan.tilesPerRow,
                            weights_[plan.kernelSize].ptr, plan.kernelSize, plan.transparent ? 1 : 0};
      CU(t360::launchGather(gp, numSMs_, s));
    }
  }

  void blurFrame(const DevicePlan* const* plans, const FramePlanes& f, PlaneLane* lanes, cudaStream_t s) {
    const FrameListRefs l = frameLists(plans, f.numPlanes);
    t360::FrameStripParams fp{};
    for (int p = 0; p < f.numPlanes; ++p) {
      const int bp = scratchPlane(lanes[p].blurred, f.inW[p], f.inH[p]);
      fp.plane[p] = {f.in[p], lanes[p].blurred.ptr, f.inW[p], f.inH[p], f.inPitch[p], bp};
    }
    launchLowPass(l.blurLayout, false, l.blurImage, l.blurImage, fp, f.numPlanes, s);
  }

  bool viewLowPass(const char* what, const FrameTransformContext& ctx, const DevicePlan* const* plans, const FramePlanes& f, StreamSlot& slot,
                   cudaStream_t s, const uint8_t** src, int* srcPitch) {
    const int numPlanes = f.numPlanes;
    const int indices = numPlanes > 1 ? 2 : 1;
    HostPlan h[2];
    std::vector<long long> key{static_cast<long long>(planGeneration_), numPlanes};
    for (int idx = 0; idx < indices; ++idx) {
      const DevicePlan& plan = *plans[idx];
      h[idx].ctx = ctx;
      h[idx].inW = plan.inW; h[idx].inH = plan.inH; h[idx].outW = plan.outW; h[idx].outH = plan.outH; h[idx].mapW = plan.mapW; h[idx].mapH = plan.mapH;
      if (!t360::buildLowPassPlan(h[idx])) {
        std::printf("%s. Error: no low-pass plan for index %d\n", what, idx);
        return false;
      }
      key.push_back(reinterpret_cast<intptr_t>(&plan));
      key.push_back(static_cast<long long>(h[idx].taps.size()));
      const std::vector<float>& taps = h[idx].taps;
      const t360::LowPassSegment* prev = nullptr;
      for (const t360::LowPassSegment& g : h[idx].segments) {
        const bool same = prev && g.kxCount == prev->kxCount && g.kyCount == prev->kyCount &&
                          std::memcmp(&taps[g.kxOffset], &taps[prev->kxOffset], sizeof(float) * g.kxCount) == 0 &&
                          std::memcmp(&taps[g.kyOffset], &taps[prev->kyOffset], sizeof(float) * g.kyCount) == 0;
        for (long long v : {g.left, g.top, g.width, g.height, g.kxOffset, g.kxCount, g.kyOffset, g.kyCount}) key.push_back(v);
        key.push_back(same);
        prev = &g;
      }
    }
    ViewBlurCache& c = slot.viewBlur;
    std::vector<uint8_t> taps;
    if (c.key == key) {
      taps.resize(c.tapCodes.size() * sizeof(float));
      float* t = reinterpret_cast<float*>(taps.data());
      for (size_t i = 0; i < c.tapCodes.size(); ++i) {
        const int code = c.tapCodes[i];
        t[i] = code ? h[(code >> t360::kTapPlaneShift) ? 1 : 0].taps[(code & ((1 << t360::kTapPlaneShift) - 1)) - 1] : 0.f;
      }
    } else {
      c = ViewBlurCache{};
      t360::BlurLists lists[2];
      for (int idx = 0; idx < indices; ++idx) {
        c.clear[idx] = plans[idx]->blur.needsClear;
        t360::buildBlurLists(h[idx].segments, h[idx].taps, plans[idx]->inW, plans[idx]->inH, plans[idx]->stereoFormat, lists[idx],
                             perFrameOnly_ ? &c.clear[idx] : nullptr);
      }
      const t360::BlurLists* perPlane[kPlaneLanes];
      bool clear[kPlaneLanes];
      for (int p = 0; p < numPlanes; ++p) {
        perPlane[p] = &lists[p ? 1 : 0];
        clear[p] = c.clear[p ? 1 : 0];
      }
      c.merged = mergeable(plans, perPlane, clear, numPlanes, f.inW, f.inH);
      auto appendCodes = [&](const t360::BlurLists& l, const t360::BlurLayout& at, int plane) {
        c.tapCodes.resize(taps.size() / sizeof(float), 0);
        for (size_t i = 0; i < l.tapSource.size(); ++i)
          c.tapCodes[at.tapAt / sizeof(float) + i] = l.tapSource[i] ? (plane << t360::kTapPlaneShift) | l.tapSource[i] : 0;
      };
      if (c.merged) {
        const t360::BlurLists all = t360::mergeBlurLists(perPlane, numPlanes);
        c.layout[0] = t360::packBlurLists(all, c.jobs, taps);
        appendCodes(all, c.layout[0], 0);
      } else {
        for (int idx = 0; idx < indices; ++idx) {
          c.layout[idx] = t360::packBlurLists(lists[idx], c.jobs, taps);
          appendCodes(lists[idx], c.layout[idx], idx);
        }
      }
      c.key = std::move(key);
    }
    UploadRing::Entry* used[2];
    const uint8_t* dJobs = stageUpload(slot.viewJobs, c.jobs, s, &used[0]);
    const uint8_t* dTaps = stageUpload(slot.viewTaps, taps, s, &used[1]);
    t360::FrameStripParams fp{};
    for (int p = 0; p < numPlanes; ++p) {
      const int bp = scratchPlane(slot.lanes[p].blurred, f.inW[p], f.inH[p]);
      src[p] = slot.lanes[p].blurred.ptr;
      srcPitch[p] = bp;
      fp.plane[p] = {f.in[p], slot.lanes[p].blurred.ptr, f.inW[p], f.inH[p], f.inPitch[p], bp};
    }
    if (c.merged) {
      launchLowPass(c.layout[0], false, dJobs, dTaps, fp, numPlanes, s);
    } else {
      for (int p = 0; p < numPlanes; ++p) {
        t360::FrameStripParams one{};
        one.plane[0] = fp.plane[p];
        launchLowPass(c.layout[p ? 1 : 0], c.clear[p ? 1 : 0], dJobs, dTaps, one, 1, s);
      }
    }
    for (UploadRing::Entry* e : used) releaseAfter(e, s);
    return true;
  }

  static const uint8_t* stageUpload(UploadRing& ring, const std::vector<uint8_t>& bytes, cudaStream_t s, UploadRing::Entry** used) {
    if (ring.last >= 0 && ring.lastContent == bytes) {
      *used = &ring.entries[ring.last];
      return ring.entries[ring.last].device;
    }
    const int i = (ring.last + 1) % UploadRing::kEntries;
    UploadRing::Entry& e = ring.entries[i];
    ring.last = -1;
    if (!e.released) CU(cudaEventCreateWithFlags(&e.released, cudaEventDisableTiming));
    if (e.inFlight) CU(cudaEventSynchronize(e.released));
    e.inFlight = false;
    if (bytes.size() > e.capacity) {
      const size_t cap = std::max<size_t>(bytes.size() + bytes.size() / 4, 4096);
      if (e.host) CU(cudaFreeHost(e.host));
      e.host = nullptr;
      if (e.device) CU(cudaFreeAsync(e.device, s));
      e.device = nullptr;
      e.capacity = 0;
      CU(cudaHostAlloc(reinterpret_cast<void**>(&e.host), cap, cudaHostAllocDefault));
      CU(cudaMallocAsync(reinterpret_cast<void**>(&e.device), cap, s));
      e.capacity = cap;
    }
    if (!bytes.empty()) {
      std::memcpy(e.host, bytes.data(), bytes.size());
      CU(cudaMemcpyAsync(e.device, e.host, bytes.size(), cudaMemcpyHostToDevice, s));
    }
    ring.last = i;
    ring.lastContent = bytes;
    *used = &e;
    return e.device;
  }

  FrameListRefs frameLists(const DevicePlan* const* plans, int numPlanes) {
    std::lock_guard<std::mutex> lock(frameListsMu_);
    FrameLists& f = frameLists_[numPlanes - 2];
    if (f.generation != planGeneration_) {
      if (f.generation != ~0ull) CU(cudaDeviceSynchronize());
      buildFrameLists(plans, numPlanes, f);
      f.generation = planGeneration_;
    }
    return FrameListRefs{f.gatherJobs.ptr, f.numGatherJobs, f.blurImage.ptr, f.blurLayout};
  }

  void buildFrameLists(const DevicePlan* const* plans, int numPlanes, FrameLists& f) {
    std::vector<GatherJob> jobs;
    const t360::BlurLists* lists[kPlaneLanes];
    for (int p = 0; p < numPlanes; ++p) {
      for (GatherJob t : plans[p]->hostJobs) {
        t.outY |= p << t360::kJobPlaneShift;
        jobs.push_back(t);
      }
      lists[p] = &plans[p]->blur.lists;
    }
    std::stable_sort(jobs.begin(), jobs.end(), [](const GatherJob& a, const GatherJob& b) { return t360::jobLaunchRank(a) < t360::jobLaunchRank(b); });
    std::vector<uint8_t> image;
    const t360::BlurLayout layout = t360::packBlurLists(t360::mergeBlurLists(lists, numPlanes), image, image);
    f.gatherJobs.reserve(jobs.size());
    if (!jobs.empty()) CU(cudaMemcpy(f.gatherJobs.ptr, jobs.data(), jobs.size() * sizeof(GatherJob), cudaMemcpyHostToDevice));
    f.blurImage.reserve(image.size());
    if (!image.empty()) CU(cudaMemcpy(f.blurImage.ptr, image.data(), image.size(), cudaMemcpyHostToDevice));
    f.numGatherJobs = static_cast<int>(jobs.size());
    f.blurLayout = layout;
  }

  void gatherFrame(const GatherWork* work, int numPlanes, cudaStream_t s, StreamSlot& slot) {
    const DevicePlan* plans[kPlaneLanes];
    for (int p = 0; p < numPlanes; ++p) plans[p] = work[p].plan;
    const FrameListRefs f = frameLists(plans, numPlanes);
    armScheduler(slot.frameClaim, s);
    t360::FrameGatherParams fp{};
    CUtensorMap maps[kPlaneLanes][t360::kMaxBoxMaps];
    for (int p = 0; p < numPlanes; ++p) {
      fp.plane[p] = work[p].view;
      std::memcpy(maps[p], work[p].maps, sizeof(work[p].maps));
    }
    fp.weightImage = reinterpret_cast<const uint4*>(weightImages_[work[0].plan->kernelSize].ptr);
    fp.kernelSize = work[0].plan->kernelSize;
    fp.numPlanes = numPlanes;
    if (traceEnabled_) {
      trace_.reserve(static_cast<size_t>(numSMs_) * t360::gatherGroups(work[0].plan->kernelSize) * t360::kTraceJobsPerGroup * 4);
      CU(cudaMemsetAsync(trace_.ptr, 0, trace_.bytes(), s));
    }
    t360::StagedParams jobs{f.gatherJobs, f.numGatherJobs, slot.frameClaim.ptr, traceEnabled_ ? trace_.ptr : nullptr};
    CU(t360::launchGatherFrame(fp, jobs, maps, numSMs_, s));
  }

  PlaneTarget renderTarget(const DevicePlan* plan, bool chroma, bool transparent, uint8_t* out, int outPitch, int outW, int outH,
                           DeviceBuffer<uint8_t>* scratch, cudaStream_t s) {
    PlaneTarget t{out, outPitch, outW, outH, out, outPitch, outW, outH, nullptr};
    if (plan && (outW != plan->mapW || outH != plan->mapH)) {
      t.resize = &resizeFor(*plan, outW, outH);
      t.dstPitch = scratchPlane(*scratch, plan->mapW, plan->mapH);
      t.dst = scratch->ptr;
      t.dstW = plan->mapW;
      t.dstH = plan->mapH;
      if (transparent) CU(cudaMemset2DAsync(t.dst, t.dstPitch, chroma ? 128 : 0, t.dstW, t.dstH, s));
    } else if (transparent && chroma) {
      CU(cudaMemset2DAsync(out, outPitch, 128, outW, outH, s));
    }
    return t;
  }

  void finishTarget(const PlaneTarget& t, cudaStream_t s) {
    if (!t.resize) return;
    const DevicePlan::Resize& r = *t.resize;
    t360::AreaParams ap{t.dst, t.out, t.dstW, t.dstH, t.dstPitch, t.outW, t.outH, t.outPitch,
                        r.cellW, r.cellH, r.xTaps.ptr, r.xFirst.ptr, r.yTaps.ptr, r.yFirst.ptr, r.xLinear.ptr, r.yLinear.ptr, r.xMax};
    CU(t360::launchAreaResize(ap, s));
  }

  struct PlanSizes { int index, inW, inH, outW, outH; };
  std::vector<PlanSizes> plannedSizes() {
    std::lock_guard<std::mutex> lock(mu_);
    std::vector<PlanSizes> sizes;
    for (const auto& kv : plans_) sizes.push_back({kv.first, kv.second.inW, kv.second.inH, kv.second.outW, kv.second.outH});
    return sizes;
  }

  bool planesOfPlannedSize(const FramePlanes& f) {
    std::lock_guard<std::mutex> lock(mu_);
    for (int p = 0; p < f.numPlanes; ++p) {
      auto it = plans_.find(p ? 1 : 0);
      if (it != plans_.end() && (f.inW[p] != it->second.inW || f.inH[p] != it->second.inH)) return false;
    }
    return true;
  }

  bool refuseWarpPlans(const char* what) {
    std::lock_guard<std::mutex> lock(mu_);
    for (const auto& kv : plans_)
      if (kv.second.warp) {
        std::printf("%s. Error: plan index %d was generated from a warp map, which has no geometry to re-plan or to move "
                    "(generateMapForPlane on the index replaces it)\n", what, kv.first);
        return true;
      }
    return false;
  }

  std::shared_lock<std::shared_mutex> lockPlanned(const char* what) {
    for (;;) {
      std::shared_lock<std::shared_mutex> config(configMu_);
      if (!perFrameOnly_) return config;
      config.unlock();
      if (reconfigureWait(true) < 0) {
        std::printf("%s. Error: the background planner failed on the current context\n", what);
        return {};
      }
    }
  }

  static const char* asyncRefusal(const FrameTransformContext& next, const std::vector<PlanSizes>& sizes) {
    if (t360::kernelSizeOf(next.interpolation_alg) == 0) return "unknown interpolation_alg";
    for (float v : {next.input_expand_coef, next.expand_coef, next.width_scale_factor, next.height_scale_factor, next.fixed_yaw,
                    next.fixed_pitch, next.fixed_roll, next.fixed_hfov, next.fixed_vfov, next.fixed_cube_offcenter_x,
                    next.fixed_cube_offcenter_y, next.fixed_cube_offcenter_z, next.kernel_height_scale_factor, next.min_kernel_half_height,
                    next.max_kernel_half_height, next.kernel_adjust_factor})
      if (!std::isfinite(v)) return "a float field is not finite";
    if (!next.enable_low_pass_filter) return nullptr;
    if (next.num_vertical_segments < 1) return "num_vertical_segments must be positive";
    for (const PlanSizes& z : sizes) {
      HostPlan h;
      h.ctx = next;
      h.inW = z.inW; h.inH = z.inH; h.outW = z.outW; h.outH = z.outH;
      h.mapW = static_cast<int>(next.width_scale_factor * z.outW + 0.5);
      h.mapH = static_cast<int>(next.height_scale_factor * z.outH + 0.5);
      if (!t360::buildLowPassPlan(h)) return "the low-pass planner refuses the context";
    }
    return nullptr;
  }

  static bool planAll(const FrameTransformContext& next, const std::vector<PlanSizes>& sizes, std::vector<HostIndexPlan>& host,
                      const char* what) {
    host.assign(sizes.size(), HostIndexPlan{});
    std::vector<int> planned(sizes.size(), 0);
    std::vector<std::string> errors(sizes.size());
    auto planOne = [&](size_t i) {
      try {
        planned[i] = planOnHost(next, sizes[i].inW, sizes[i].inH, sizes[i].outW, sizes[i].outH, host[i]);
      } catch (const std::exception& ex) {
        errors[i] = ex.what();
      }
    };
    std::vector<std::thread> pool;
    for (size_t i = 1; i < sizes.size(); ++i) pool.emplace_back(planOne, i);
    planOne(0);
    for (std::thread& t : pool) t.join();
    for (size_t i = 0; i < sizes.size(); ++i)
      if (!planned[i]) {
        std::printf("%s. Error: no plan for index %d%s%s\n", what, sizes[i].index, errors[i].empty() ? "" : ": ", errors[i].c_str());
        return false;
      }
    return true;
  }

  struct PlanSet {
    std::map<int, DevicePlan> plans;
    FrameLists lists[kPlaneLanes - 1];
    std::vector<PlaneGraph> graphs;
  };
  PlanSet makePlanSet(const FrameTransformContext& next, const std::vector<PlanSizes>& sizes, std::vector<HostIndexPlan>& host) {
    PlanSet set;
    for (size_t i = 0; i < sizes.size(); ++i) set.plans.emplace(sizes[i].index, upload(host[i], next));
    auto luma = set.plans.find(0), chroma = set.plans.find(1);
    if (luma != set.plans.end() && chroma != set.plans.end()) {
      const DevicePlan* planes[kPlaneLanes] = {&luma->second, &chroma->second, &chroma->second};
      for (int n = 2; n <= kPlaneLanes; ++n) {
        buildFrameLists(planes, n, set.lists[n - 2]);
        set.lists[n - 2].generation = planGeneration_ + 1;
      }
    }
    return set;
  }

  bool install(PlanSet& set, const FrameTransformContext& next, unsigned long long seq, bool evenIfSuperseded) {
    std::unique_lock<std::shared_mutex> config(configMu_);
    std::lock_guard<std::mutex> async(asyncMu_);
    const bool current = asyncSeq_ == seq;
    if (!current && !evenIfSuperseded) return false;
    {
      std::lock_guard<std::mutex> lock(mu_);
      std::lock_guard<std::mutex> listsLock(frameListsMu_);
      plans_.swap(set.plans);
      for (int i = 0; i < kPlaneLanes - 1; ++i) std::swap(frameLists_[i], set.lists[i]);
      set.graphs.swap(planeGraphs_);
      ++planGeneration_;
    }
    if (current) {
      std::memcpy(&ctx_, &next, sizeof(ctx_));
      perFrameOnly_ = false;
      asyncSettled_ = seq;
      asyncFailed_ = false;
      asyncCv_.notify_all();
    }
    return true;
  }

  void retire(PlanSet& old) {
// ... 421 lines not shown
  return t->transformFrameWith(what, *orientation, f, static_cast<cudaStream_t>(stream));
}
T360_API int T360B200_orientedSamples(const FrameTransformContext* ctx, const T360Orientation* orientation, int inW, int inH, int outW,
                                      int outH, int32_t* samples) {
  return perFrameSamples("orientation", ctx, orientation, inW, inH, outW, outH, samples);
}
T360_API int T360B200_transformFramePoseAsync(VideoFrameTransform* t, const T360Pose* pose, int numPlanes, const uint8_t* const* dIn,
                                              uint8_t* const* dOut, const int* inW, const int* inH, const int* inPitch, const int* outW,
                                              const int* outH, const int* outPitch, void* stream) {
  const char* what = "Could not transform the frame with a pose";
  FramePlanes f;
  if (!t || !pose || !describeFrame(what, numPlanes, dIn, dOut, inW, inH, inPitch, outW, outH, outPitch, f)) return 0;
  return t->transformFrameWith(what, *pose, f, static_cast<cudaStream_t>(stream));
}
T360_API int T360B200_poseSamples(const FrameTransformContext* ctx, const T360Pose* pose, int inW, int inH, int outW, int outH, int32_t* samples) {
  return perFrameSamples("pose", ctx, pose, inW, inH, outW, outH, samples);
}
T360_API int T360B200_remapFrameAsync(VideoFrameTransform* t, int numPlanes, const float* const* maps, const int* mapPitches, int border,
                                      const uint8_t* const* dIn, uint8_t* const* dOut, const int* inW, const int* inH, const int* inPitch,
                                      const int* outW, const int* outH, const int* outPitch, void* stream) {
  const char* what = "Could not remap the frame";
  if (!t || !maps || !mapPitches) {
    std::printf("%s. Error: a NULL argument\n", what);
    return 0;
  }
  FramePlanes f;
  if (!describeFrame(what, numPlanes, dIn, dOut, inW, inH, inPitch, outW, outH, outPitch, f)) return 0;
  return t->remapFrame(maps, mapPitches, border, f, static_cast<cudaStream_t>(stream));
}
T360_API int T360B200_lensMap(const FrameTransformContext* ctx, const T360LensRig* rig, const T360Orientation* orientation, int inW, int inH,
                              int outW, int outH, float* map) {
  const char* what = "Could not compute the lens map";
  std::string why;
  if (!ctx) why = "a NULL context";
  else if (lensRefused(*ctx, rig, orientation, &why)) {}
  else if (!map || inW <= 0 || inH <= 0 || outW <= 0 || outH <= 0) why = "a NULL map or a plane size that is not positive";
  if (!why.empty()) {
    std::printf("%s. Error: %s\n", what, why.c_str());
    return 0;
  }
  const t360::LensRigModel model = lensRigModel(*rig);
  forLensPixels(*ctx, *orientation, inW, inH, outW, outH, [&](const t360::SphereGeometry& g, const t360::Rotation& r, const float* colTab,
                                                              const float* rowTab, int i, int j, size_t at) {
    t360::lensPoint(g, r, model, colTab, rowTab, i, j, map + 2 * at, map + 2 * at + 1);
  });
  return 1;
}
T360_API int T360B200_lensBlendMaps(const FrameTransformContext* ctx, const T360LensRig* rig, float seamWidth, const T360Orientation* orientation,
                                    int inW, int inH, int outW, int outH, float* map0, float* map1, uint16_t* weight) {
  const char* what = "Could not compute the lens blend maps";
  std::string why;
  if (!ctx) why = "a NULL context";
  else if (lensBlendRefused(*ctx, rig, seamWidth, orientation, &why)) {}
  else if (!map0 || !map1 || !weight || inW <= 0 || inH <= 0 || outW <= 0 || outH <= 0)
    why = "a NULL map or weight array or a plane size that is not positive";
  if (!why.empty()) {
    std::printf("%s. Error: %s\n", what, why.c_str());
    return 0;
  }
  const t360::LensRigModel model = lensRigModel(*rig);
  const float s = lensSeamScale(seamWidth);
  forLensPixels(*ctx, *orientation, inW, inH, outW, outH, [&](const t360::SphereGeometry& g, const t360::Rotation& r, const float* colTab,
                                                              const float* rowTab, int i, int j, size_t at) {
    weight[at] = static_cast<uint16_t>(t360::lensBlendPoint(g, r, model, s, colTab, rowTab, i, j, map0 + 2 * at, map1 + 2 * at));
  });
  return 1;
}
T360_API int T360B200_transformFrameLensAsync(VideoFrameTransform* t, const T360LensRig* rig, const T360Orientation* orientation, int numPlanes,
                                              const uint8_t* const* dIn, uint8_t* const* dOut, const int* inW, const int* inH, const int* inPitch,
                                              const int* outW, const int* outH, const int* outPitch, void* stream) {
  const char* what = "Could not transform the frame with a lens rig";
  if (!t) {
    std::printf("%s. Error: a NULL argument\n", what);
    return 0;
  }
  FramePlanes f;
  if (!describeFrame(what, numPlanes, dIn, dOut, inW, inH, inPitch, outW, outH, outPitch, f)) return 0;
  return t->transformFrameLens(what, rig, nullptr, orientation, f, static_cast<cudaStream_t>(stream));
}
T360_API int T360B200_transformFrameLensBlendAsync(VideoFrameTransform* t, const T360LensRig* rig, float seamWidth, const T360Orientation* orientation,
                                                   int numPlanes, const uint8_t* const* dIn, uint8_t* const* dOut, const int* inW, const int* inH,
                                                   const int* inPitch, const int* outW, const int* outH, const int* outPitch, void* stream) {
  const char* what = "Could not blend the frame of a lens rig";
  if (!t) {
    std::printf("%s. Error: a NULL argument\n", what);
    return 0;
  }
  FramePlanes f;
  if (!describeFrame(what, numPlanes, dIn, dOut, inW, inH, inPitch, outW, outH, outPitch, f)) return 0;
  return t->transformFrameLens(what, rig, &seamWidth, orientation, f, static_cast<cudaStream_t>(stream));
}
namespace {
int cameraMap(const char* what, const FrameTransformContext* ctx, const T360LensRig* rig, const T360Pose* pose, const T360Camera* camera,
              int inW, int inH, int outW, int outH, float* map) {
  std::string why;
  if (!ctx) why = "a NULL context";
  else if (cameraRefused(*ctx, rig, pose, camera, &why)) {}
  else if (!map || inW <= 0 || inH <= 0 || outW <= 0 || outH <= 0) why = "a NULL map or a plane size that is not positive";
  if (!why.empty()) {
    std::printf("%s. Error: %s\n", what, why.c_str());
    return 0;
  }
  const t360::SphereGeometry g = rectilinearGeometry(*ctx, rig != nullptr, inW, inH, outW, outH);
  const t360::RectilinearCamera c = cameraConstants(*pose, *camera);
  const t360::LensRigModel model = rig ? lensRigModel(*rig) : t360::LensRigModel{};
  for (int i = 0; i < outH; ++i)
    for (int j = 0; j < outW; ++j) {
      float* at = map + 2 * (static_cast<size_t>(i) * outW + j);
      if (rig) t360::rectilinearPosition<true>(g, c, model, i, j, at, at + 1);
      else t360::rectilinearPosition<false>(g, c, model, i, j, at, at + 1);
    }
  return 1;
}
int transformFrameCamera(const char* what, VideoFrameTransform* t, const T360LensRig* rig, const T360Pose* pose, const T360Camera* camera,
                         int numPlanes, const uint8_t* const* dIn, uint8_t* const* dOut, const int* inW, const int* inH, const int* inPitch,
                         const int* outW, const int* outH, const int* outPitch, void* stream) {
  if (!t) {
    std::printf("%s. Error: a NULL argument\n", what);
    return 0;
  }
  FramePlanes f;
  if (!describeFrame(what, numPlanes, dIn, dOut, inW, inH, inPitch, outW, outH, outPitch, f)) return 0;
  return t->transformFrameCamera(what, rig, pose, camera, f, static_cast<cudaStream_t>(stream));
}
}
T360_API int T360B200_cameraMap(const FrameTransformContext* ctx, const T360LensRig* rig, const T360Pose* pose, const T360Camera* camera, int inW,
                                int inH, int outW, int outH, float* map) {
  return cameraMap("Could not compute the camera map", ctx, rig, pose, camera, inW, inH, outW, outH, map);
}
T360_API int T360B200_transformFrameCameraAsync(VideoFrameTransform* t, const T360LensRig* rig, const T360Pose* pose, const T360Camera* camera,
                                                int numPlanes, const uint8_t* const* dIn, uint8_t* const* dOut, const int* inW, const int* inH,
                                                const int* inPitch, const int* outW, const int* outH, const int* outPitch, void* stream) {
  return transformFrameCamera("Could not transform the frame with a camera view", t, rig, pose, camera, numPlanes, dIn, dOut, inW, inH, inPitch,
                              outW, outH, outPitch, stream);
}
T360_API int T360B200_rectilinearMap(const FrameTransformContext* ctx, const T360LensRig* rig, const T360Pose* pose, int inW, int inH, int outW,
                                     int outH, float* map) {
  return cameraMap("Could not compute the rectilinear map", ctx, rig, pose, &kPinhole, inW, inH, outW, outH, map);
}
T360_API int T360B200_transformFrameRectilinearAsync(VideoFrameTransform* t, const T360LensRig* rig, const T360Pose* pose, int numPlanes,
                                                     const uint8_t* const* dIn, uint8_t* const* dOut, const int* inW, const int* inH,
                                                     const int* inPitch, const int* outW, const int* outH, const int* outPitch, void* stream) {
  return transformFrameCamera("Could not transform the frame with a rectilinear view", t, rig, pose, &kPinhole, numPlanes, dIn, dOut, inW, inH,
                              inPitch, outW, outH, outPitch, stream);
}
T360_API void T360B200_setPinHostPlanes(VideoFrameTransform* t, int enable) { if (t) t->setPinHostPlanes(enable != 0); }
T360_API void T360B200_debugTrace(VideoFrameTransform* t, int enable) { if (t) t->enableTrace(enable != 0); }
T360_API unsigned long long T360B200_debugTraceRead(VideoFrameTransform* t, unsigned long long* out, unsigned long long maxWords) {
  return t ? t->readTrace(out, maxWords) : 0;
}
T360_API int T360B200_synchronize(VideoFrameTransform* t) { return t ? t->synchronize() : 0; }
T360_API void* T360B200_stream(VideoFrameTransform* t) { return t ? t->stream() : nullptr; }
T360_API unsigned long long T360B200_kernelLaunchCount(void) { return t360::kernelLaunchCount(); }
T360_API unsigned long long T360B200_planDeviceBytes(VideoFrameTransform* t, int planIndex) { return t ? t->planBytes(planIndex) : 0; }
T360_API int T360B200_planTileCounts(VideoFrameTransform* t, int planIndex, int counts[4]) {
  return t && counts ? t->tileCounts(planIndex, counts) : 0;
}
T360_API int T360B200_deviceCount(void) {
  int n = 0;
  if (cudaGetDeviceCount(&n) != cudaSuccess) {
    cudaGetLastError();
    return 0;
  }
  return n;
}
T360_API const char* T360B200_version(void) { return "transform360-b200 0.1 (sm_90a)"; }
```

### transform360_b200/handler.py

```python
from __future__ import annotations

import ctypes as C
import os
from pathlib import Path

import numpy as np

PKG = Path(__file__).resolve().parent
LIB_PATH = PKG / "lib" / "libTransform360.so"

LAYOUT_CUBEMAP_32, LAYOUT_CUBEMAP_23_OFFCENTER, LAYOUT_FLAT_FIXED, LAYOUT_EQUIRECT = 0, 1, 2, 3
LAYOUT_BARREL, LAYOUT_BARREL_SPLIT, LAYOUT_EAC_32, LAYOUT_N = 4, 5, 6, 7
STEREO_FORMAT_TB, STEREO_FORMAT_LR, STEREO_FORMAT_MONO, STEREO_FORMAT_GUESS, STEREO_FORMAT_N = 0, 1, 2, 3, 4
NEAREST, LINEAR, CUBIC, LANCZOS4 = 0, 1, 2, 4
BORDER_WRAP, BORDER_TRANSPARENT = 3, 5


def _warp_map(map) -> np.ndarray:
    m = np.ascontiguousarray(map, np.float32)
    if m.ndim != 3 or m.shape[2] != 2:
        raise ValueError(f"a warp map is float32 [h][w][2] (x, y per output pixel), got shape {m.shape}")
    return m


# ... 58 lines not shown


def as_orientation(orientation) -> T360Orientation:
    if isinstance(orientation, T360Orientation):
        return orientation
    return T360Orientation(*[float(v) for v in orientation])


class T360Pose(C.Structure):
    _fields_ = [("yaw", C.c_float), ("pitch", C.c_float), ("roll", C.c_float), ("hfov", C.c_float), ("vfov", C.c_float)]


def as_pose(pose) -> T360Pose:
    return pose if isinstance(pose, T360Pose) else T360Pose(*[float(v) for v in pose])


T360_CAMERA_PINHOLE, T360_CAMERA_EQUIDISTANT, T360_CAMERA_STEREOGRAPHIC, T360_CAMERA_PANNINI = 0, 1, 2, 3


class T360Camera(C.Structure):
    _fields_ = [("model", C.c_int), ("pannini", C.c_float)]


def as_camera(camera) -> T360Camera:
    if isinstance(camera, T360Camera):
        return camera
    if isinstance(camera, (tuple, list)):
        return T360Camera(int(camera[0]), float(camera[1]))
    return T360Camera(int(camera), 0.0)


class T360Lens(C.Structure):
    _fields_ = [("fx", C.c_float), ("fy", C.c_float), ("cx", C.c_float), ("cy", C.c_float), ("k", C.c_float * 4),
                ("yaw", C.c_float), ("pitch", C.c_float), ("roll", C.c_float), ("maxAngle", C.c_float)]


class T360LensRig(C.Structure):
    _fields_ = [("numLenses", C.c_int), ("calibWidth", C.c_int), ("calibHeight", C.c_int), ("lens", T360Lens * 2)]


def make_context(**overrides) -> FrameTransformContext:
    vals = dict(FILTER_DEFAULTS)
    for k in overrides:
        if k not in vals:
            raise AttributeError(f"FrameTransformContext has no field {k!r}")
    vals.update(overrides)
    return FrameTransformContext(**vals)


_lib = None


def load(path: os.PathLike | None = None):
    global _lib
    if _lib is not None and path is None:
        return _lib
    p = Path(path) if path else Path(os.environ.get("T360B200_LIB") or LIB_PATH)
    if not p.exists():
        raise FileNotFoundError(f"{p} not found: build it with `python -m transform360_b200.build` (needs nvcc); "
                                "transform360_b200 has no CPU fallback")
    L = C.CDLL(str(p), mode=os.RTLD_LOCAL)
    vp, ci = C.c_void_p, C.c_int
    planes = [vp, vp] + [vp] * 6 + [vp]
    L.VideoFrameTransform_new.restype = vp
    L.VideoFrameTransform_new.argtypes = [C.POINTER(FrameTransformContext)]
    L.VideoFrameTransform_delete.restype = None
    L.VideoFrameTransform_delete.argtypes = [vp]
    L.VideoFrameTransform_generateMapForPlane.restype = ci
    L.VideoFrameTransform_generateMapForPlane.argtypes = [vp] + [ci] * 5
    L.VideoFrameTransform_transformFramePlane.restype = ci
    L.VideoFrameTransform_transformFramePlane.argtypes = [vp, vp, vp] + [ci] * 8
    L.T360B200_hostPlanCreate.restype = vp
    L.T360B200_hostPlanCreate.argtypes = [C.POINTER(FrameTransformContext)] + [ci] * 4
    L.T360B200_hostPlanCreateFromWarp.restype = vp
    L.T360B200_hostPlanCreateFromWarp.argtypes = [C.POINTER(FrameTransformContext), vp] + [ci] * 5
    L.T360B200_generateMapFromWarp.restype = ci
    L.T360B200_generateMapFromWarp.argtypes = [vp, vp] + [ci] * 6
    L.T360B200_remapFrameAsync.restype = ci
    L.T360B200_remapFrameAsync.argtypes = [vp, ci, vp, vp, ci] + planes
    L.T360B200_hostPlanDestroy.restype = None
    L.T360B200_hostPlanDestroy.argtypes = [vp]
    L.T360B200_hostPlanInfo.restype = ci
    L.T360B200_hostPlanInfo.argtypes = [vp, C.POINTER(ci)]
    L.T360B200_hostPlanMap.restype = vp
    L.T360B200_hostPlanMap.argtypes = [vp]
    L.T360B200_hostPlanSamples.restype = vp
    L.T360B200_hostPlanSamples.argtypes = [vp]
    L.T360B200_hostPlanSegment.restype = ci
    L.T360B200_hostPlanSegment.argtypes = [vp, ci, C.POINTER(ci), C.POINTER(ci), C.POINTER(vp), C.POINTER(vp)]
    L.T360B200_hostPlanGather.restype = ci
    L.T360B200_hostPlanGather.argtypes = [vp, C.POINTER(ci), C.POINTER(vp), C.POINTER(vp), C.POINTER(vp)]
    L.T360B200_hostPlanPoleCaps.restype = ci
    L.T360B200_hostPlanBlurLists.restype = ci
    L.T360B200_hostPlanBlurLists.argtypes = [vp, ci, ci, ci, C.POINTER(ci), C.POINTER(vp)]
    L.T360B200_hostPlanPoleCaps.argtypes = [vp, C.POINTER(ci), C.POINTER(vp), C.POINTER(vp), C.POINTER(vp)]
    L.T360B200_hostPlanDeviceLists.restype = ci
    L.T360B200_hostPlanDeviceLists.argtypes = [vp, C.POINTER(ci), C.POINTER(vp), C.POINTER(vp)]
    L.T360B200_weightImage.restype = ci
    L.T360B200_weightImage.argtypes = [ci, C.POINTER(vp)]
    L.T360B200_remapTable.restype = ci
    L.T360B200_remapTable.argtypes = [ci, C.POINTER(vp)]
    L.T360B200_transformFramePlaneAsync.restype = ci
    L.T360B200_transformFramePlaneAsync.argtypes = [vp, vp, vp] + [ci] * 7 + [vp]
    L.T360B200_transformFrameAsync.restype = ci
    L.T360B200_transformFrameAsync.argtypes = [vp, ci] + planes
    L.T360B200_lowPassPlaneAsync.restype = ci
    L.T360B200_lowPassPlaneAsync.argtypes = [vp, vp, vp] + [ci] * 5 + [vp]
    L.T360B200_reconfigure.restype = ci
    L.T360B200_reconfigure.argtypes = [vp, C.POINTER(FrameTransformContext)]
    L.T360B200_reconfigureAsync.restype = ci
    L.T360B200_reconfigureAsync.argtypes = [vp, C.POINTER(FrameTransformContext)]
    L.T360B200_reconfigureWait.restype = ci
    L.T360B200_reconfigureWait.argtypes = [vp, ci]
    L.T360B200_transformFrameViewAsync.restype = ci
    L.T360B200_transformFrameViewAsync.argtypes = [vp, C.POINTER(T360View), ci] + planes
    L.T360B200_viewSamples.restype = ci
    L.T360B200_viewSamples.argtypes = [C.POINTER(FrameTransformContext), C.POINTER(T360View)] + [ci] * 4 + [vp]
    L.T360B200_transformFrameOrientedAsync.restype = ci
    L.T360B200_transformFrameOrientedAsync.argtypes = [vp, C.POINTER(T360Orientation), ci] + planes
    L.T360B200_orientedSamples.restype = ci
    L.T360B200_orientedSamples.argtypes = [C.POINTER(FrameTransformContext), C.POINTER(T360Orientation)] + [ci] * 4 + [vp]
    L.T360B200_transformFramePoseAsync.restype = ci
    L.T360B200_transformFramePoseAsync.argtypes = [vp, C.POINTER(T360Pose), ci] + planes
    L.T360B200_poseSamples.restype = ci
    L.T360B200_poseSamples.argtypes = [C.POINTER(FrameTransformContext), C.POINTER(T360Pose)] + [ci] * 4 + [vp]
    L.T360B200_lensMap.restype = ci
    L.T360B200_lensMap.argtypes = [C.POINTER(FrameTransformContext), C.POINTER(T360LensRig), C.POINTER(T360Orientation)] + [ci] * 4 + [vp]
    L.T360B200_transformFrameLensAsync.restype = ci
    L.T360B200_transformFrameLensAsync.argtypes = [vp, C.POINTER(T360LensRig), C.POINTER(T360Orientation), ci] + planes
    L.T360B200_lensBlendMaps.restype = ci
    L.T360B200_lensBlendMaps.argtypes = [C.POINTER(FrameTransformContext), C.POINTER(T360LensRig), C.c_float, C.POINTER(T360Orientation)] + [ci] * 4 + [vp] * 3
    L.T360B200_transformFrameLensBlendAsync.restype = ci
    L.T360B200_transformFrameLensBlendAsync.argtypes = [vp, C.POINTER(T360LensRig), C.c_float, C.POINTER(T360Orientation), ci] + planes
    L.T360B200_rectilinearMap.restype = ci
    L.T360B200_rectilinearMap.argtypes = [C.POINTER(FrameTransformContext), C.POINTER(T360LensRig), C.POINTER(T360Pose)] + [ci] * 4 + [vp]
    L.T360B200_transformFrameRectilinearAsync.restype = ci
    L.T360B200_transformFrameRectilinearAsync.argtypes = [vp, C.POINTER(T360LensRig), C.POINTER(T360Pose), ci] + planes
    L.T360B200_cameraMap.restype = ci
    L.T360B200_cameraMap.argtypes = [C.POINTER(FrameTransformContext), C.POINTER(T360LensRig), C.POINTER(T360Pose),
                                     C.POINTER(T360Camera)] + [ci] * 4 + [vp]
    L.T360B200_transformFrameCameraAsync.restype = ci
    L.T360B200_transformFrameCameraAsync.argtypes = [vp, C.POINTER(T360LensRig), C.POINTER(T360Pose), C.POINTER(T360Camera), ci] + planes
    L.T360B200_setPinHostPlanes.restype = None
    L.T360B200_setPinHostPlanes.argtypes = [vp, ci]
    L.T360B200_debugTrace.restype = None
    L.T360B200_debugTrace.argtypes = [vp, ci]
    L.T360B200_debugTraceRead.restype = C.c_ulonglong
    L.T360B200_debugTraceRead.argtypes = [vp, vp, C.c_ulonglong]
    L.T360B200_synchronize.restype = ci
    L.T360B200_synchronize.argtypes = [vp]
    L.T360B200_stream.restype = vp
    L.T360B200_stream.argtypes = [vp]
    L.T360B200_kernelLaunchCount.restype = C.c_ulonglong
    L.T360B200_planDeviceBytes.restype = C.c_ulonglong
    L.T360B200_planDeviceBytes.argtypes = [vp, ci]
    L.T360B200_planTileCounts.restype = ci
    L.T360B200_planTileCounts.argtypes = [vp, ci, C.POINTER(ci)]
    L.T360B200_deviceCount.restype = ci
    L.T360B200_version.restype = C.c_char_p
    if path is None:
        _lib = L
    return L


EXPORTED_SYMBOLS = [
    "VideoFrameTransform_new", "VideoFrameTransform_delete", "VideoFrameTransform_generateMapForPlane",
    "VideoFrameTransform_transformFramePlane", "T360B200_hostPlanCreate", "T360B200_hostPlanCreateFromWarp", "T360B200_hostPlanDestroy",
    "T360B200_generateMapFromWarp", "T360B200_remapFrameAsync",
    "T360B200_hostPlanInfo", "T360B200_hostPlanMap", "T360B200_hostPlanSamples", "T360B200_hostPlanSegment",
    "T360B200_hostPlanGather", "T360B200_hostPlanPoleCaps", "T360B200_hostPlanDeviceLists", "T360B200_hostPlanBlurLists", "T360B200_weightImage", "T360B200_dealLanes",
    "T360B200_remapTable", "T360B200_transformFramePlaneAsync", "T360B200_transformFrameAsync",
    "T360B200_lowPassPlaneAsync", "T360B200_reconfigure", "T360B200_reconfigureAsync", "T360B200_reconfigureWait",
    "T360B200_transformFrameViewAsync", "T360B200_viewSamples",
    "T360B200_transformFrameOrientedAsync", "T360B200_orientedSamples", "T360B200_transformFramePoseAsync", "T360B200_poseSamples",
    "T360B200_lensMap", "T360B200_transformFrameLensAsync", "T360B200_lensBlendMaps", "T360B200_transformFrameLensBlendAsync",
    "T360B200_rectilinearMap", "T360B200_transformFrameRectilinearAsync", "T360B200_cameraMap", "T360B200_transformFrameCameraAsync",
    "T360B200_setPinHostPlanes", "T360B200_debugTrace", "T360B200_debugTraceRead", "T360B200_synchronize", "T360B200_stream", "T360B200_kernelLaunchCount", "T360B200_planDeviceBytes",
    "T360B200_planTileCounts", "T360B200_deviceCount", "T360B200_version",
]


class VideoFrameTransform:

    def __init__(self, ctx: FrameTransformContext):
        self._lib = load()
        self.ctx = ctx
        self._h = self._lib.VideoFrameTransform_new(C.byref(ctx))
        if not self._h:
            raise MemoryError("VideoFrameTransform_new returned NULL")

    def close(self):
        if getattr(self, "_h", None):
            self._lib.VideoFrameTransform_delete(self._h)
            self._h = None

    __del__ = close

    def __enter__(self):
        return self

    def __exit__(self, *exc):
        self.close()

    def generateMapForPlane(self, inputWidth, inputHeight, outputWidth, outputHeight, transformMatPlaneIndex) -> bool:
        return bool(self._lib.VideoFrameTransform_generateMapForPlane(
            self._h, inputWidth, inputHeight, outputWidth, outputHeight, transformMatPlaneIndex))

    def transformFramePlane(self, inputData, outputData, inputWidth, inputHeight, inputWidthWithPadding,
                            outputWidth, outputHeight, outputWidthWithPadding, transformMatPlaneIndex,
                            imagePlaneIndex) -> bool:
        return bool(self._lib.VideoFrameTransform_transformFramePlane(
            self._h, inputData, outputData, inputWidth, inputHeight, inputWidthWithPadding, outputWidth,
            outputHeight, outputWidthWithPadding, transformMatPlaneIndex, imagePlaneIndex))

    def transform_plane(self, src: np.ndarray, out_w: int, out_h: int, plan_index: int, image_plane: int = 0,
                        out: np.ndarray | None = None) -> np.ndarray:
        assert src.dtype == np.uint8 and src.ndim == 2 and src.strides[1] == 1
        if out is None:
            out = np.zeros((out_h, out_w), np.uint8)
        assert out.dtype == np.uint8 and out.shape == (out_h, out_w) and out.strides[1] == 1
        ok = self.transformFramePlane(src.ctypes.data, out.ctypes.data, src.shape[1], src.shape[0], src.strides[0],
                                      out_w, out_h, out.strides[0], plan_index, image_plane)
        if not ok:
            raise RuntimeError("VideoFrameTransform_transformFramePlane returned 0 (message on stdout)")
        return out

    def transform_plane_async(self, d_in: int, d_out: int, in_w, in_h, in_pitch, out_w, out_h, out_pitch, plan_index,
                              stream: int = 0) -> bool:
        return bool(self._lib.T360B200_transformFramePlaneAsync(self._h, d_in, d_out, in_w, in_h, in_pitch, out_w,
                                                                out_h, out_pitch, plan_index, stream))

    def _frame_call(self, entry: str, in_planes, out_planes, dims):
        n, pin, pout, ptrs, keep = _frame_args(in_planes, out_planes, dims)
        fn, h = getattr(self._lib, entry), self._h

        def enqueue(lead, stream, _keep=keep) -> bool:
            return bool(fn(h, *lead, pin, pout, *ptrs, stream))
        return n, enqueue

    def make_frame_call(self, in_planes, out_planes, dims):
        n, enqueue = self._frame_call("T360B200_transformFrameAsync", in_planes, out_planes, dims)
        return lambda stream=0: enqueue((n,), stream)

    def make_view_frame_call(self, in_planes, out_planes, dims):
        n, enqueue = self._frame_call("T360B200_transformFrameViewAsync", in_planes, out_planes, dims)
        return lambda view, stream=0: enqueue((C.byref(as_view(view)), n), stream)

    def make_oriented_frame_call(self, in_planes, out_planes, dims):
        n, enqueue = self._frame_call("T360B200_transformFrameOrientedAsync", in_planes, out_planes, dims)
        return lambda orientation, stream=0: enqueue((C.byref(as_orientation(orientation)), n), stream)

    def make_pose_frame_call(self, in_planes, out_planes, dims):
        n, enqueue = self._frame_call("T360B200_transformFramePoseAsync", in_planes, out_planes, dims)
        return lambda pose, stream=0: enqueue((C.byref(as_pose(pose)), n), stream)

    def make_lens_frame_call(self, in_planes, out_planes, dims):
        n, enqueue = self._frame_call("T360B200_transformFrameLensAsync", in_planes, out_planes, dims)
        return lambda rig, orientation, stream=0: enqueue((C.byref(rig), C.byref(as_orientation(orientation)), n), stream)

    def make_lens_blend_frame_call(self, in_planes, out_planes, dims):
        n, enqueue = self._frame_call("T360B200_transformFrameLensBlendAsync", in_planes, out_planes, dims)
        return lambda rig, seam_width, orientation, stream=0: enqueue(
            (C.byref(rig), seam_width, C.byref(as_orientation(orientation)), n), stream)

    def make_rectilinear_frame_call(self, in_planes, out_planes, dims):
        n, enqueue = self._frame_call("T360B200_transformFrameRectilinearAsync", in_planes, out_planes, dims)
        return lambda pose, stream=0, rig=None: enqueue((C.byref(rig) if rig is not None else None, C.byref(as_pose(pose)), n), stream)

    def make_camera_frame_call(self, in_planes, out_planes, dims):
        n, enqueue = self._frame_call("T360B200_transformFrameCameraAsync", in_planes, out_planes, dims)
        return lambda pose, camera, stream=0, rig=None: enqueue(
            (C.byref(rig) if rig is not None else None, C.byref(as_pose(pose)), C.byref(as_camera(camera)), n), stream)

    def generate_map_from_warp(self, map, in_w: int, in_h: int, plan_index: int, border: int = BORDER_WRAP) -> bool:
        m = _warp_map(map)
        return bool(self._lib.T360B200_generateMapFromWarp(self._h, m.ctypes.data, m.shape[1], m.shape[0], in_w, in_h, border,
                                                           plan_index))

    def make_remap_frame_call(self, in_planes, out_planes, dims, border: int = BORDER_WRAP):
        n, enqueue = self._frame_call("T360B200_remapFrameAsync", in_planes, out_planes, dims)
        dense = [8 * d[2] for d in dims]

        def as_map(m, p):
            if hasattr(m, "data_ptr"):
                return m.data_ptr(), m.stride(0) * m.element_size()
            return (int(m[0]), int(m[1])) if isinstance(m, (tuple, list)) else (int(m), dense[p])

        def call(maps, stream: int = 0) -> bool:
            if len(maps) != n:
                raise ValueError(f"{len(maps)} maps for {n} planes")
            desc = [as_map(m, p) for p, m in enumerate(maps)]
            dmaps, pitches = (C.c_void_p * n)(*[d[0] for d in desc]), (C.c_int * n)(*[d[1] for d in desc])
            return enqueue((n, dmaps, pitches, border), stream)
        return call

    def low_pass_async(self, d_in: int, d_out: int, w, h, in_pitch, out_pitch, plan_index, stream: int = 0) -> bool:
        return bool(self._lib.T360B200_lowPassPlaneAsync(self._h, d_in, d_out, w, h, in_pitch, out_pitch, plan_index,
                                                         stream))

    def reconfigure(self, ctx: FrameTransformContext) -> None:
        if not self._lib.T360B200_reconfigure(self._h, C.byref(ctx)):
            raise RuntimeError("T360B200_reconfigure returned 0 (message on stdout); the old configuration is still in effect")
        self.ctx = ctx

    def reconfigure_async(self, ctx: FrameTransformContext) -> None:
        if not self._lib.T360B200_reconfigureAsync(self._h, C.byref(ctx)):
            raise RuntimeError("T360B200_reconfigureAsync returned 0 (message on stdout); the old context is still in effect")
        self.ctx = ctx

    def reconfigure_wait(self, block: bool = True) -> int:
        return self._lib.T360B200_reconfigureWait(self._h, 1 if block else 0)

    def set_pin_host_planes(self, enable: bool) -> None:
        self._lib.T360B200_setPinHostPlanes(self._h, 1 if enable else 0)

    def debug_trace(self, enable: bool) -> None:
        self._lib.T360B200_debugTrace(self._h, 1 if enable else 0)

    def read_trace(self) -> np.ndarray:
        buf = np.zeros(int(self._lib.T360B200_debugTraceRead(self._h, None, 0)), np.uint64)
        n = int(self._lib.T360B200_debugTraceRead(self._h, buf.ctypes.data, buf.size)) if buf.size else 0
        return buf[:n].reshape(-1, 64, 4)

    def synchronize(self) -> bool:
        return bool(self._lib.T360B200_synchronize(self._h))

    @property
    def stream(self) -> int:
        return self._lib.T360B200_stream(self._h) or 0

# ... 37 lines not shown
    def map(self) -> np.ndarray:
        p = self._lib.T360B200_hostPlanMap(self._h)
        n = self.map_w * self.map_h * 2
        return np.frombuffer((C.c_float * n).from_address(p), np.float32).reshape(self.map_h, self.map_w, 2).copy()

    @property
    def samples(self) -> np.ndarray:
        p = self._lib.T360B200_hostPlanSamples(self._h)
        n = self.map_w * self.map_h * 2
        return np.frombuffer((C.c_int32 * n).from_address(p), np.int32).reshape(self.map_h, self.map_w, 2).copy()

    def gather_plan(self):
        info = (C.c_int * 10)()
        jobs, recs, comp = C.c_void_p(), C.c_void_p(), C.c_void_p()
        if not self._lib.T360B200_hostPlanGather(self._h, info, C.byref(jobs), C.byref(recs), C.byref(comp)):
            raise ValueError("T360B200_hostPlanGather failed")
        tpr, trows, th, nj = info[0], info[1], info[2], info[3]
        n = tpr * trows * th * 32 * 2
        records = np.frombuffer((C.c_int32 * n).from_address(recs.value), np.int32).reshape(tpr * trows, th, 32, 2).copy()
        j = compact = None
        if nj and jobs.value:
            j = np.frombuffer((C.c_int32 * (nj * 4)).from_address(jobs.value), np.int32).reshape(nj, 4).copy()
        if info[9] and comp.value:
            compact = np.frombuffer((C.c_uint32 * info[9]).from_address(comp.value), np.uint32).copy()
        return dict(tiles_per_row=tpr, tile_rows=trows, tile_h=th, jobs=j, records=records, compact=compact,
                    counts=dict(class0=info[4], class1=info[5], seam=info[6], general=info[7], share=info[8]))

    def pole_caps(self):
        info = (C.c_int * 4)()
        jobs, recs, launch = C.c_void_p(), C.c_void_p(), C.c_void_p()
        if not self._lib.T360B200_hostPlanPoleCaps(self._h, info, C.byref(jobs), C.byref(recs), C.byref(launch)):
            raise ValueError("T360B200_hostPlanPoleCaps failed")
        n, m = info[0] + info[1], info[3]
        as_jobs = lambda p, k: np.frombuffer((C.c_int32 * (k * 4)).from_address(p.value), np.int32).reshape(k, 4).copy() if k and p.value else np.zeros((0, 4), np.int32)
        records = np.frombuffer((C.c_uint32 * info[2]).from_address(recs.value), np.uint32).copy() if info[2] and recs.value else np.zeros(0, np.uint32)
        return dict(counts=dict(cap=info[0], border=info[1]), jobs=as_jobs(jobs, n), records=records, launch=as_jobs(launch, m))

    def device_lists(self):
        info = (C.c_int * 2)()
        jobs, recs = C.c_void_p(), C.c_void_p()
        if not self._lib.T360B200_hostPlanDeviceLists(self._h, info, C.byref(jobs), C.byref(recs)):
            raise ValueError("T360B200_hostPlanDeviceLists failed")
        j = np.frombuffer((C.c_int32 * (info[0] * 4)).from_address(jobs.value), np.int32).reshape(-1, 4).copy() if info[0] and jobs.value else np.zeros((0, 4), np.int32)
        r = np.frombuffer((C.c_uint32 * info[1]).from_address(recs.value), np.uint32).copy() if info[1] and recs.value else np.zeros(0, np.uint32)
        return dict(jobs=j, records=r)

    def blur_lists(self, *others, width=0, height=0):
        plans = (C.c_void_p * (1 + len(others)))(self._h, *[o._h for o in others])
        lay, img = (C.c_int * 15)(), C.c_void_p()
        if not self._lib.T360B200_hostPlanBlurLists(plans, len(plans), width, height, lay, C.byref(img)):
            raise ValueError("T360B200_hostPlanBlurLists failed (message on stdout)")
        image = C.string_at(img.value, lay[14]) if lay[14] else b""
        arr = lambda at, n, cols, dt: np.frombuffer(image, dt, n * cols, at).reshape(n, cols).copy()
        return dict(image=image, strips=[arr(lay[8 + c], lay[c], 9, np.int32) for c in range(3)], tiles=arr(lay[11], lay[3], 8, np.int32),
                    direct=arr(lay[12], lay[4], 8, np.int32), taps=np.frombuffer(image, np.float32, lay[5], lay[13]).copy(),
                    offsets=list(lay[8:14]), tile_smem=lay[6], needs_clear=bool(lay[7]))

    def segments(self):
        out = []
        rect, nk = (C.c_int * 4)(), (C.c_int * 2)()
        kx, ky = C.c_void_p(), C.c_void_p()
        for i in range(self.num_segments):
            assert self._lib.T360B200_hostPlanSegment(self._h, i, rect, nk, C.byref(kx), C.byref(ky))
            a = np.frombuffer((C.c_float * nk[0]).from_address(kx.value), np.float32).copy()
            b = np.frombuffer((C.c_float * nk[1]).from_address(ky.value), np.float32).copy()
            out.append((rect[0], rect[1], rect[2], rect[3], a, b))
        return out


def view_samples(ctx: FrameTransformContext, view, in_w, in_h, out_w, out_h) -> np.ndarray:
    return _samples(load().T360B200_viewSamples, ctx, as_view(view), in_w, in_h, out_w, out_h)


def oriented_samples(ctx: FrameTransformContext, orientation, in_w, in_h, out_w, out_h) -> np.ndarray:
    return _samples(load().T360B200_orientedSamples, ctx, as_orientation(orientation), in_w, in_h, out_w, out_h)


def pose_samples(ctx: FrameTransformContext, pose, in_w, in_h, out_w, out_h) -> np.ndarray:
    return _samples(load().T360B200_poseSamples, ctx, as_pose(pose), in_w, in_h, out_w, out_h)


def lens_map(ctx: FrameTransformContext, rig: T360LensRig, orientation, in_w, in_h, out_w, out_h) -> np.ndarray:
    out = np.zeros((max(out_h, 0), max(out_w, 0), 2), np.float32)
    if not load().T360B200_lensMap(C.byref(ctx), C.byref(rig), C.byref(as_orientation(orientation)), in_w, in_h, out_w, out_h,
                                   out.ctypes.data):
        raise ValueError("T360B200_lensMap refused the arguments (message on stdout)")
    return out


def lens_blend_maps(ctx: FrameTransformContext, rig: T360LensRig, seam_width, orientation, in_w, in_h, out_w,
                    out_h) -> tuple[np.ndarray, np.ndarray, np.ndarray]:
    shape = (max(out_h, 0), max(out_w, 0))
    map0, map1, weight = np.zeros(shape + (2,), np.float32), np.zeros(shape + (2,), np.float32), np.zeros(shape, np.uint16)
    if not load().T360B200_lensBlendMaps(C.byref(ctx), C.byref(rig), seam_width, C.byref(as_orientation(orientation)), in_w, in_h,
                                         out_w, out_h, map0.ctypes.data, map1.ctypes.data, weight.ctypes.data):
        raise ValueError("T360B200_lensBlendMaps refused the arguments (message on stdout)")
    return map0, map1, weight


def rectilinear_map(ctx: FrameTransformContext, pose, in_w, in_h, out_w, out_h, rig: T360LensRig | None = None) -> np.ndarray:
    out = np.zeros((max(out_h, 0), max(out_w, 0), 2), np.float32)
    if not load().T360B200_rectilinearMap(C.byref(ctx), C.byref(rig) if rig is not None else None, C.byref(as_pose(pose)), in_w, in_h,
                                          out_w, out_h, out.ctypes.data):
        raise ValueError("T360B200_rectilinearMap refused the arguments (message on stdout)")
    return out


def camera_map(ctx: FrameTransformContext, pose, camera, in_w, in_h, out_w, out_h, rig: T360LensRig | None = None) -> np.ndarray:
    out = np.zeros((max(out_h, 0), max(out_w, 0), 2), np.float32)
    if not load().T360B200_cameraMap(C.byref(ctx), C.byref(rig) if rig is not None else None, C.byref(as_pose(pose)),
                                     C.byref(as_camera(camera)), in_w, in_h, out_w, out_h, out.ctypes.data):
        raise ValueError("T360B200_cameraMap refused the arguments (message on stdout)")
    return out


def square_pixel_vfov(hfov, width, height) -> float:
    return float(np.degrees(2.0 * np.arctan(np.tan(np.radians(hfov) / 2.0) * height / width)))


def remap_table(interpolation_alg: int) -> np.ndarray | None:
    L = load()
    p = C.c_void_p()
    k = L.T360B200_remapTable(interpolation_alg, C.byref(p))
    if k < 2:
        return None
    return np.frombuffer((C.c_int16 * (1024 * k * k)).from_address(p.value), np.int16).reshape(1024, k, k).copy()


def deal_lanes(interpolation_alg: int, phases) -> tuple[int, np.ndarray, np.ndarray]:
    L = load()
    ph = np.ascontiguousarray(phases, np.int32)
    lane, copy = np.zeros(ph.size, np.int32), np.zeros(ph.size, np.int32)
    L.T360B200_dealLanes.restype = C.c_int
    L.T360B200_dealLanes.argtypes = [C.c_int, C.c_int, C.c_void_p, C.c_void_p, C.c_void_p]
    w = L.T360B200_dealLanes(interpolation_alg, ph.size, ph.ctypes.data, lane.ctypes.data, copy.ctypes.data)
    if w < 0:
        raise ValueError("T360B200_dealLanes refused the arguments")
    return int(w), lane, copy


def weight_image(interpolation_alg: int) -> np.ndarray | None:
    L = load()
    p = C.c_void_p()
    n = L.T360B200_weightImage(interpolation_alg, C.byref(p))
    if n <= 0:
        return None
    return np.frombuffer((C.c_uint8 * n).from_address(p.value), np.uint8).copy()


def kernel_launch_count() -> int:
    return int(load().T360B200_kernelLaunchCount())


def device_count() -> int:
    return int(load().T360B200_deviceCount())
```

Baseline: 761,100.

## Stage gather tile outputs in shared memory and write them with TMA stores

Output pixels of class0/class1 tile jobs are now written byte by byte into a per-warp shared-memory staging buffer and sent to global memory with a 2D TMA bulk tensor store, instead of scattered byte stores straight to global memory. The staging buffers are multi-buffered per stage, with bulk wait_group.read guarding reuse. Tiles with skipped records, and seam, cap and border jobs, still store directly. This is meant to replace uncoalesced u8 global stores with bulk async writes, at the cost of more shared memory per CTA and extra fences and syncs. The staged path is enabled only for kernel sizes other than 8, which includes bicubic (K=4).

```diff
diff --git a/include/transform360_b200.h b/include/transform360_b200.h
--- a/include/transform360_b200.h
+++ b/include/transform360_b200.h
@@ -131,6 +131,7 @@
 void* T360B200_stream(VideoFrameTransform* transform);
 
 unsigned long long T360B200_kernelLaunchCount(void);
+unsigned long long T360B200_stagedStoreLaunchCount(void);
 unsigned long long T360B200_planDeviceBytes(VideoFrameTransform* transform, int transformMatPlaneIndex);
 int T360B200_planTileCounts(VideoFrameTransform* transform, int transformMatPlaneIndex, int counts[4]);
 int T360B200_deviceCount(void);
diff --git a/transform360_b200/__init__.py b/transform360_b200/__init__.py
--- a/transform360_b200/__init__.py
+++ b/transform360_b200/__init__.py
@@ -4,4 +4,4 @@
                       T360_CAMERA_PINHOLE, T360_CAMERA_STEREOGRAPHIC,
                       FrameTransformContext, HostPlan, T360Camera, T360Lens, T360LensRig, T360Orientation, T360Pose, T360View, VideoFrameTransform, device_count, kernel_launch_count,
                       camera_map, lens_blend_maps, lens_map, load, make_context, oriented_samples, pose_samples, rectilinear_map, remap_table,
-                      square_pixel_vfov, view_samples, weight_image, deal_lanes)
+                      square_pixel_vfov, staged_store_launch_count, view_samples, weight_image, deal_lanes)
diff --git a/transform360_b200/csrc/gather_frame.cu b/transform360_b200/csrc/gather_frame.cu
--- a/transform360_b200/csrc/gather_frame.cu
+++ b/transform360_b200/csrc/gather_frame.cu
@@ -68,6 +68,25 @@
 __device__ __forceinline__ void groupBarrier(int group) {
   asm volatile("bar.sync %0, %1;" ::"r"(group + 1), "n"(kGroupThreads) : "memory");
 }
+__device__ __forceinline__ void tmaStoreBox(const CUtensorMap* map, uint32_t src, int x, int y) {
+  asm volatile("cp.async.bulk.tensor.2d.global.shared::cta.bulk_group [%0, {%1, %2}], [%3];"
+               ::"l"(reinterpret_cast<uint64_t>(map)), "r"(x), "r"(y), "r"(src) : "memory");
+  asm volatile("cp.async.bulk.commit_group;" ::: "memory");
+}
+template <int N>
+__device__ __forceinline__ void bulkWaitRead() { asm volatile("cp.async.bulk.wait_group.read %0;" ::"n"(N) : "memory"); }
+
+struct GlobalOut {
+  uint8_t* p;
+  int pitch;
+  __device__ __forceinline__ void put(int row, int col, uint32_t v) const { p[(size_t)row * pitch + col] = (uint8_t)v; }
+};
+struct SharedOut {
+  uint32_t a;
+  __device__ __forceinline__ void put(int row, int col, uint32_t v) const {
+    asm volatile("st.shared.u8 [%0], %1;" ::"r"(a + (uint32_t)(row * kOutStageW + col)), "r"(v) : "memory");
+  }
+};
 
 template <int K>
 struct RowBytes {
@@ -203,13 +222,12 @@
   });
 }
 
-template <int K, int PITCH, int VS>
+template <int K, int PITCH, int VS, class Out>
 __device__ __forceinline__ void computeTileJob(const PlaneView& pv, uint32_t stageAddr, int outX, int outY, const uint4& rec,
-                                               uint32_t wAddr, int warp) {
+                                               uint32_t wAddr, int warp, const Out& out) {
   static_assert(PITCH % 4 == 0, "");
   const int y0 = outY + warp * kTilePatchH;
-  const int dstPitch = pv.dstPitch, dstW = pv.dstW, dstH = pv.dstH;
-  uint8_t* const dstRow = pv.dst + (size_t)y0 * dstPitch + outX;
+  const int dstW = pv.dstW, dstH = pv.dstH;
   const uint32_t words[4] = {rec.x, rec.y, rec.z, rec.w};
   staticFor<kRowsPerPatchStep>([&](auto J) {
     constexpr int j = decltype(J)::value;
@@ -221,7 +239,7 @@
       RowBytes<K> W[K];
       staticFor<K>([&](auto R) { W[decltype(R)::value] = loadRow<K, decltype(R)::value * PITCH>(rowAddr, sh); });
       const int acc = foldPixel<K, VS>(W, wAddr, (w >> 17) & kSlotFieldMask);
-      dstRow[(size_t)row * dstPitch + col] = (uint8_t)biasedToByte(acc);
+      out.put(row, col, (uint32_t)biasedToByte(acc));
     }
   });
 }
@@ -259,6 +277,7 @@
 template <int K>
 struct FrameTensorMaps {
   CUtensorMap map[kMaxFramePlanes][boxMaps(K)];
+  CUtensorMap out[kMaxFramePlanes];
 };
 
 __device__ __forceinline__ void mbarArrive(uint64_t* bar) {
@@ -275,7 +294,7 @@
   return v;
 }
 
-template <int K, int COPIES, int GROUPS>
+template <int K, int COPIES, int GROUPS, bool STORE>
 struct FrameLayout {
   static constexpr int kStages = gatherStages(K);
   static constexpr int kWeights = weightImageBytes(K, COPIES);
@@ -283,16 +302,19 @@
   static constexpr int kGroupBytes = kStages * (kStage + kRec);
   static constexpr int kPlanes = kWeights + GROUPS * kGroupBytes;
   static constexpr int kBars = kPlanes + 256;
-  static constexpr int kTotal = kBars + GROUPS * kStages * 16 + 16;
+  static constexpr int kOut = (kBars + GROUPS * kStages * 16 + 16 + 127) & ~127;
+  static constexpr int kOutStage = kOutStageW * kTilePatchH;
+  static constexpr int kTotal = STORE ? kOut + GROUPS * kStages * kGroupWarps * kOutStage : kBars + GROUPS * kStages * 16 + 16;
   static_assert(kTotal <= 232448, "227 KB of shared memory per CTA");
+  static_assert(kOutStage % 128 == 0, "TMA store sources");
   static_assert(sizeof(PlaneView) * kMaxFramePlanes <= 256, "");
   static_assert(kStage % 128 == 0 && kRec % 128 == 0 && kWeights % 128 == 0, "TMA / bulk-copy destinations");
 };
 
-template <int K, int COPIES, int GROUPS>
+template <int K, int COPIES, int GROUPS, bool STORE>
 __global__ void __launch_bounds__(GROUPS * (kGroupWarps + 1) * 32, 1)
 gatherFrameKernel(const __grid_constant__ FrameGatherParams p, StagedParams jobs, const __grid_constant__ FrameTensorMaps<K> maps) {
-  using L = FrameLayout<K, COPIES, GROUPS>;
+  using L = FrameLayout<K, COPIES, GROUPS, STORE>;
   constexpr int VS = weightVectorStride(K, COPIES), kStage = L::kStage, kRec = L::kRec, S = L::kStages;
   constexpr uint32_t kBox0 = stageBoxW(K, 0) * stageBoxH(K, 0), kBox1 = stageBoxW(K, 1) * stageBoxH(K, 1),
                      kBoxShare = stageBoxW(K, 2) * stageBoxH(K, 2);
@@ -412,6 +434,22 @@
   const uint32_t wAddr = smemAddr(wsmem);
   mbarWait(weightBar, 0);
   asm volatile("griddepcontrol.wait;" ::: "memory");
+  const uint32_t outAddr = smemAddr(smem + L::kOut) + (uint32_t)(((group * S) * kGroupWarps + warp) * L::kOutStage);
+  int lastStore = -1;
+  auto stagingBuffer = [&](uint32_t st) {
+    if (lane == 0) {
+      if (lastStore == (int)st) bulkWaitRead<0>();
+      else bulkWaitRead<1>();
+    }
+    __syncwarp();
+    return SharedOut{outAddr + st * (kGroupWarps * L::kOutStage)};
+  };
+  auto storeStaged = [&](uint32_t st, int pl, int x, int y) {
+    asm volatile("fence.proxy.async.shared::cta;" ::: "memory");
+    __syncwarp();
+    if (lane == 0) tmaStoreBox(&maps.out[pl], outAddr + st * (kGroupWarps * L::kOutStage), x, y);
+    lastStore = (int)st;
+  };
   auto now = []() { unsigned long long t; asm volatile("mov.u64 %0, %globaltimer;" : "=l"(t)); return t; };
   unsigned long long* trace = jobs.trace && warp == 0 && lane == 0 ? jobs.trace + (size_t)(blockIdx.x * GROUPS + group) * kTraceJobsPerGroup * 4 : nullptr;
   uint32_t traced = 0;
@@ -426,6 +464,16 @@
     if (kind == kJobExit) break;
     const int outX = (int)h.x & ~kJobQuadMask, outY = (int)h.y & kJobRowMask;
     const PlaneView& pv = planes[(int)h.y >> kJobPlaneShift];
+    auto tileJob = [&](const uint4& r, auto&& compute) {
+      if constexpr (STORE) {
+        if (__all_sync(0xffffffffu, ((r.x | r.y | r.z | r.w) & kRecordSkip) == 0)) {
+          compute(stagingBuffer(st));
+          storeStaged(st, (int)h.y >> kJobPlaneShift, outX, outY + warp * kTilePatchH);
+          return;
+        }
+      }
+      compute(GlobalOut{pv.dst + (size_t)(outY + warp * kTilePatchH) * pv.dstPitch + outX, pv.dstPitch});
+    };
     if (kind == kJobShare || kind == kJobShareStay) {
       if constexpr (K >= 4) {
         const uint32_t mine = rec + 128 + warp * shareWarpRecordBytes(K);
@@ -450,12 +498,15 @@
         }
       }
       const int width = (int)(h.w >> kJobWidthShift);
-      staticFor<class0Widths(K)>([&](auto W) {
-        constexpr int w = decltype(W)::value;
-        if (width == w) computeTileJob<K, class0BoxW(w), VS>(pv, boxAddr + st * kStage, outX, outY, r, wAddr, warp);
+      tileJob(r, [&](const auto& out) {
+        staticFor<class0Widths(K)>([&](auto W) {
+          constexpr int w = decltype(W)::value;
+          if (width == w) computeTileJob<K, class0BoxW(w), VS>(pv, boxAddr + st * kStage, outX, outY, r, wAddr, warp, out);
+        });
       });
     } else if (kind == kJobClass1) {
-      computeTileJob<K, stageBoxW(K, 1), VS>(pv, boxAddr + st * kStage, outX, outY, ldsVec(rec + 128 + warp * 512 + lane * 16), wAddr, warp);
+      const uint4 r = ldsVec(rec + 128 + warp * 512 + lane * 16);
+      tileJob(r, [&](const auto& out) { computeTileJob<K, stageBoxW(K, 1), VS>(pv, boxAddr + st * kStage, outX, outY, r, wAddr, warp, out); });
     } else if (kind == kJobSeam) {
       {
         uint4* a = reinterpret_cast<uint4*>(groupBase + st * kStage);
@@ -469,7 +520,8 @@
         asm volatile("fence.proxy.async.shared::cta;" ::: "memory");
       }
       groupBarrier(group);
-      computeTileJob<K, stageBoxW(K, 0), VS>(pv, boxAddr + st * kStage, outX, outY, ldsVec(rec + 128 + warp * 512 + lane * 16), wAddr, warp);
+      computeTileJob<K, stageBoxW(K, 0), VS>(pv, boxAddr + st * kStage, outX, outY, ldsVec(rec + 128 + warp * 512 + lane * 16), wAddr, warp,
+                                             GlobalOut{pv.dst + (size_t)(outY + warp * kTilePatchH) * pv.dstPitch + outX, pv.dstPitch});
     } else if (kind == kJobCap) {
       computeCapJob<K, stageBoxW(K, 0), VS>(pv, boxAddr + st * kStage, rec + 128, (int)h.x, wAddr, warp, lane);
     } else if (kind == kJobBorder) {
@@ -483,25 +535,33 @@
     }
     if (++st == S) { st = 0; phase ^= 1; }
   }
-}
-
-template <int K, int COPIES, int GROUPS>
+  if constexpr (STORE) {
+    if (lane == 0) asm volatile("cp.async.bulk.wait_group 0;" ::: "memory");
+  }
+}
+
+template <int K, int COPIES, int GROUPS, bool STORE>
 cudaError_t prepareFrameK(LaunchCfg& cfg) {
   static DeviceLaunchCfg cfgs;
-  constexpr int threads = GROUPS * (kGroupWarps + 1) * 32, smemBytes = FrameLayout<K, COPIES, GROUPS>::kTotal;
-  return prepare<gatherFrameKernel<K, COPIES, GROUPS>>(cfgs, threads, smemBytes, cfg);
-}
-
-template <int K, int COPIES, int GROUPS>
-cudaError_t launchFrameK(const FrameGatherParams& p, const StagedParams& jobs, const void* tensorMaps, int numSMs,
-                         cudaStream_t stream, bool programmatic) {
+  constexpr int threads = GROUPS * (kGroupWarps + 1) * 32, smemBytes = FrameLayout<K, COPIES, GROUPS, STORE>::kTotal;
+  return prepare<gatherFrameKernel<K, COPIES, GROUPS, STORE>>(cfgs, threads, smemBytes, cfg);
+}
+
+std::atomic<unsigned long long> gStagedStoreLaunches{0};
+
+template <int K, int COPIES, int GROUPS, bool STORE>
+cudaError_t launchFrameK(const FrameGatherParams& p, const StagedParams& jobs, const void* tensorMaps, const void* outMaps,
+                         int numSMs, cudaStream_t stream, bool programmatic) {
   FrameTensorMaps<K> maps;
-  for (int i = 0; i < kMaxFramePlanes; ++i)
-    std::memcpy(maps.map[i], static_cast<const CUtensorMap*>(tensorMaps) + (size_t)(i < p.numPlanes ? i : 0) * kMaxBoxMaps,
-                sizeof(maps.map[i]));
-  constexpr int threads = GROUPS * (kGroupWarps + 1) * 32, smemBytes = FrameLayout<K, COPIES, GROUPS>::kTotal;
+  for (int i = 0; i < kMaxFramePlanes; ++i) {
+    const size_t from = (size_t)(i < p.numPlanes ? i : 0);
+    std::memcpy(maps.map[i], static_cast<const CUtensorMap*>(tensorMaps) + from * kMaxBoxMaps, sizeof(maps.map[i]));
+    if (STORE) std::memcpy(&maps.out[i], static_cast<const CUtensorMap*>(outMaps) + from, sizeof(maps.out[i]));
+    else std::memset(&maps.out[i], 0, sizeof(maps.out[i]));
+  }
+  constexpr int threads = GROUPS * (kGroupWarps + 1) * 32, smemBytes = FrameLayout<K, COPIES, GROUPS, STORE>::kTotal;
   LaunchCfg cfg;
-  cudaError_t err = prepareFrameK<K, COPIES, GROUPS>(cfg);
+  cudaError_t err = prepareFrameK<K, COPIES, GROUPS, STORE>(cfg);
   if (err != cudaSuccess) return err;
   const int grid = std::min(numSMs * cfg.perSM, (jobs.numTiles + GROUPS * 2 - 1) / (GROUPS * 2));
   cudaLaunchConfig_t lc{};
@@ -514,33 +574,54 @@
   attr.val.programmaticStreamSerializationAllowed = 1;
   lc.attrs = &attr;
   lc.numAttrs = programmatic ? 1 : 0;
-  err = cudaLaunchKernelEx(&lc, gatherFrameKernel<K, COPIES, GROUPS>, p, jobs, maps);
+  err = cudaLaunchKernelEx(&lc, gatherFrameKernel<K, COPIES, GROUPS, STORE>, p, jobs, maps);
   gLaunches.fetch_add(1, std::memory_order_relaxed);
+  if (STORE) gStagedStoreLaunches.fetch_add(1, std::memory_order_relaxed);
   return err;
 }
 
+template <int K>
+cudaError_t prepareFrame() {
+  LaunchCfg cfg;
+  cudaError_t err = prepareFrameK<K, weightCopies(K), gatherGroups(K), false>(cfg);
+  if constexpr (stagedTileStores(K)) {
+    if (err == cudaSuccess) err = prepareFrameK<K, weightCopies(K), gatherGroups(K), true>(cfg);
+  }
+  return err;
+}
+
+template <int K>
+cudaError_t launchFrame(const FrameGatherParams& p, const StagedParams& jobs, const void* tensorMaps, const void* outMaps, int numSMs,
+                        cudaStream_t stream, bool programmatic) {
+  if constexpr (stagedTileStores(K)) {
+    if (outMaps) return launchFrameK<K, weightCopies(K), gatherGroups(K), true>(p, jobs, tensorMaps, outMaps, numSMs, stream, programmatic);
+  }
+  return launchFrameK<K, weightCopies(K), gatherGroups(K), false>(p, jobs, tensorMaps, outMaps, numSMs, stream, programmatic);
+}
+
 }
 
 cudaError_t prepareGatherFrame(int kernelSize) {
-  LaunchCfg cfg;
   switch (kernelSize) {
-    case 2: return prepareFrameK<2, weightCopies(2), gatherGroups(2)>(cfg);
-    case 4: return prepareFrameK<4, weightCopies(4), gatherGroups(4)>(cfg);
-    case 8: return prepareFrameK<8, weightCopies(8), gatherGroups(8)>(cfg);
+    case 2: return prepareFrame<2>();
+    case 4: return prepareFrame<4>();
+    case 8: return prepareFrame<8>();
     default: return cudaErrorInvalidValue;
   }
 }
 
-cudaError_t launchGatherFrame(const FrameGatherParams& p, const StagedParams& jobs, const void* tensorMaps, int numSMs,
-                              cudaStream_t stream, bool programmatic) {
+cudaError_t launchGatherFrame(const FrameGatherParams& p, const StagedParams& jobs, const void* tensorMaps, const void* outMaps,
+                              int numSMs, cudaStream_t stream, bool programmatic) {
   if (jobs.numTiles <= 0) return cudaSuccess;
   if (p.numPlanes < 1 || p.numPlanes > kMaxFramePlanes) return cudaErrorInvalidValue;
   switch (p.kernelSize) {
-    case 2: return launchFrameK<2, weightCopies(2), gatherGroups(2)>(p, jobs, tensorMaps, numSMs, stream, programmatic);
-    case 4: return launchFrameK<4, weightCopies(4), gatherGroups(4)>(p, jobs, tensorMaps, numSMs, stream, programmatic);
-    case 8: return launchFrameK<8, weightCopies(8), gatherGroups(8)>(p, jobs, tensorMaps, numSMs, stream, programmatic);
+    case 2: return launchFrame<2>(p, jobs, tensorMaps, outMaps, numSMs, stream, programmatic);
+    case 4: return launchFrame<4>(p, jobs, tensorMaps, outMaps, numSMs, stream, programmatic);
+    case 8: return launchFrame<8>(p, jobs, tensorMaps, outMaps, numSMs, stream, programmatic);
     default: return cudaErrorInvalidValue;
   }
 }
 
-}
+unsigned long long stagedStoreLaunchCount() { return gStagedStoreLaunches.load(std::memory_order_relaxed); }
+
+}
diff --git a/transform360_b200/csrc/kernels.cuh b/transform360_b200/csrc/kernels.cuh
--- a/transform360_b200/csrc/kernels.cuh
+++ b/transform360_b200/csrc/kernels.cuh
@@ -141,6 +141,8 @@
   const uint4* weightImage;
   int kernelSize, numPlanes;
 };
+constexpr int kOutStageW = 32;
+__host__ __device__ constexpr bool stagedTileStores(int k) { return k != 8; }
 
 __host__ __device__ constexpr int gatherThreads(int k) { return k == 8 ? 512 : 256; }
 __host__ __device__ constexpr int gatherTileH(int k) { return gatherThreads(k) / 32 * 4; }
@@ -218,9 +220,10 @@
 constexpr int kBlurMaxSmem = 96 * 1024;
 
 cudaError_t launchGather(const GatherParams& p, int numSMs, cudaStream_t stream);
-cudaError_t launchGatherFrame(const FrameGatherParams& p, const StagedParams& jobs, const void* tensorMaps, int numSMs,
-                              cudaStream_t stream, bool programmatic = true);
+cudaError_t launchGatherFrame(const FrameGatherParams& p, const StagedParams& jobs, const void* tensorMaps, const void* outMaps,
+                              int numSMs, cudaStream_t stream, bool programmatic = true);
 cudaError_t prepareGatherFrame(int kernelSize);
+unsigned long long stagedStoreLaunchCount();
 cudaError_t launchBlur(const BlurParams& p, cudaStream_t stream);
 cudaError_t launchBlurDirect(const BlurParams& p, cudaStream_t stream);
 unsigned long long kernelLaunchCount();
diff --git a/transform360_b200/csrc/video_frame_transform.cpp b/transform360_b200/csrc/video_frame_transform.cpp
--- a/transform360_b200/csrc/video_frame_transform.cpp
+++ b/transform360_b200/csrc/video_frame_transform.cpp
@@ -175,13 +175,13 @@
   return fn;
 }
 
-bool encodePlaneMap(CUtensorMap* map, const uint8_t* base, int w, int h, int pitch, int k, int index) {
+bool encodePlaneMap(CUtensorMap* map, const uint8_t* base, int w, int h, int pitch, int boxW, int boxH) {
   EncodeTiledFn enc = tensorMapEncoder();
   if (!enc) return false;
   if ((reinterpret_cast<uintptr_t>(base) & 15) || (pitch & 15)) return false;
   const cuuint64_t dims[2] = {static_cast<cuuint64_t>(w), static_cast<cuuint64_t>(h)};
   const cuuint64_t strides[1] = {static_cast<cuuint64_t>(pitch)};
-  const cuuint32_t box[2] = {static_cast<cuuint32_t>(t360::boxMapW(k, index)), static_cast<cuuint32_t>(t360::boxMapRows(k, index))};
+  const cuuint32_t box[2] = {static_cast<cuuint32_t>(boxW), static_cast<cuuint32_t>(boxH)};
   const cuuint32_t elem[2] = {1, 1};
   return enc(map, CU_TENSOR_MAP_DATA_TYPE_UINT8, 2, const_cast<uint8_t*>(base), dims, strides, box, elem,
              CU_TENSOR_MAP_INTERLEAVE_NONE, CU_TENSOR_MAP_SWIZZLE_NONE, CU_TENSOR_MAP_L2_PROMOTION_L2_128B,
@@ -195,10 +195,17 @@
   int w = 0, h = 0, pitch = 0, k = 0;
   CUtensorMap maps[t360::kMaxBoxMaps];
 };
+struct OutputMap {
+  const uint8_t* base = nullptr;
+  int w = 0, h = 0, pitch = 0;
+  CUtensorMap map;
+};
 struct PlaneLane {
   static constexpr int kMapCache = 32;
   PlaneMaps mapCache[kMapCache];
   int mapCacheNext = 0;
+  OutputMap outCache[kMapCache];
+  int outCacheNext = 0;
   cudaStream_t main = nullptr;
   cudaEvent_t done = nullptr;
   DeviceBuffer<uint8_t> blurred;
@@ -219,6 +226,8 @@
   t360::PlaneView view{};
   bool staged = false;
   CUtensorMap maps[t360::kMaxBoxMaps];
+  bool storeStaged = false;
+  CUtensorMap outMap;
   PlaneTarget target;
 };
 
@@ -958,7 +967,8 @@
         const int n = w.waveStart[c + 1] - w.waveStart[c];
         if (n > 0) {
           t360::StagedParams jobs{w.jobs.ptr + w.waveStart[c], n, hostLane.claimCounter.ptr, nullptr};
-          CU(t360::launchGatherFrame(fp, jobs, work.maps, numSMs_, stream_, false));
+          CU(t360::launchGatherFrame(fp, jobs, work.maps, work.storeStaged ? &work.outMap : nullptr, numSMs_, stream_,
+                                     false));
         }
         if (!w.rects[c].empty()) {
           CU(cudaEventRecord(waveDone_[c], stream_));
@@ -1553,11 +1563,26 @@
       }
     PlaneMaps fresh;
     for (int m = 0; m < t360::boxMaps(k); ++m)
-      if (!encodePlaneMap(&fresh.maps[m], src, w, h, pitch, k, m)) return false;
+      if (!encodePlaneMap(&fresh.maps[m], src, w, h, pitch, t360::boxMapW(k, m), t360::boxMapRows(k, m))) return false;
     fresh.base = src; fresh.w = w; fresh.h = h; fresh.pitch = pitch; fresh.k = k;
     lane.mapCache[lane.mapCacheNext] = fresh;
     lane.mapCacheNext = (lane.mapCacheNext + 1) % PlaneLane::kMapCache;
     std::memcpy(out, fresh.maps, sizeof(fresh.maps));
+    return true;
+  }
+
+  static bool outputMap(PlaneLane& lane, const uint8_t* dst, int w, int h, int pitch, CUtensorMap& out) {
+    for (const OutputMap& e : lane.outCache)
+      if (e.base == dst && e.w == w && e.h == h && e.pitch == pitch) {
+        out = e.map;
+        return true;
+      }
+    OutputMap fresh;
+    if (!encodePlaneMap(&fresh.map, dst, w, h, pitch, t360::kOutStageW, t360::kTilePatchH)) return false;
+    fresh.base = dst; fresh.w = w; fresh.h = h; fresh.pitch = pitch;
+    lane.outCache[lane.outCacheNext] = fresh;
+    lane.outCacheNext = (lane.outCacheNext + 1) % PlaneLane::kMapCache;
+    out = fresh.map;
     return true;
   }
 
@@ -1590,6 +1615,7 @@
     w.view = t360::PlaneView{src, t.dst, reinterpret_cast<const uint4*>(plan.records.ptr), inW, inH, srcPitch, t.dstW, t.dstH, t.dstPitch};
     w.staged = plan.numJobs > 0 && !plan.transparent && inW == plan.inW && inH == plan.inH;
     if (w.staged) w.staged = planeMaps(lane, src, inW, inH, srcPitch, plan.kernelSize, w.maps);
+    w.storeStaged = w.staged && t360::stagedTileStores(plan.kernelSize) && outputMap(lane, t.dst, t.dstW, t.dstH, t.dstPitch, w.outMap);
     return true;
   }
 
@@ -1609,7 +1635,7 @@
       fp.kernelSize = plan.kernelSize;
       fp.numPlanes = 1;
       t360::StagedParams jobs{plan.gatherJobs.ptr, plan.numJobs, lane.claimCounter.ptr, nullptr};
-      CU(t360::launchGatherFrame(fp, jobs, w.maps, numSMs_, s));
+      CU(t360::launchGatherFrame(fp, jobs, w.maps, w.storeStaged ? &w.outMap : nullptr, numSMs_, s));
     } else {
       const t360::PlaneView& v = w.view;
       t360::GatherParams gp{v.src, v.srcW, v.srcH, v.srcPitch, v.dst, v.dstW, v.dstH, v.dstPitch, plan.samples.ptr, plan.tilesPerRow,
@@ -1789,10 +1815,13 @@
     const FrameListRefs f = frameLists(plans, numPlanes);
     armScheduler(slot.frameClaim, s);
     t360::FrameGatherParams fp{};
-    CUtensorMap maps[kPlaneLanes][t360::kMaxBoxMaps];
+    CUtensorMap maps[kPlaneLanes][t360::kMaxBoxMaps], outMaps[kPlaneLanes];
+    bool storeStaged = true;
     for (int p = 0; p < numPlanes; ++p) {
       fp.plane[p] = work[p].view;
       std::memcpy(maps[p], work[p].maps, sizeof(work[p].maps));
+      outMaps[p] = work[p].outMap;
+      storeStaged = storeStaged && work[p].storeStaged;
     }
     fp.weightImage = reinterpret_cast<const uint4*>(weightImages_[work[0].plan->kernelSize].ptr);
     fp.kernelSize = work[0].plan->kernelSize;
@@ -1802,7 +1831,7 @@
       CU(cudaMemsetAsync(trace_.ptr, 0, trace_.bytes(), s));
     }
     t360::StagedParams jobs{f.gatherJobs, f.numGatherJobs, slot.frameClaim.ptr, traceEnabled_ ? trace_.ptr : nullptr};
-    CU(t360::launchGatherFrame(fp, jobs, maps, numSMs_, s));
+    CU(t360::launchGatherFrame(fp, jobs, maps, storeStaged ? outMaps : nullptr, numSMs_, s));
   }
 
   PlaneTarget renderTarget(const DevicePlan* plan, bool chroma, bool transparent, uint8_t* out, int outPitch, int outW, int outH,
@@ -2530,6 +2559,7 @@
 T360_API int T360B200_synchronize(VideoFrameTransform* t) { return t ? t->synchronize() : 0; }
 T360_API void* T360B200_stream(VideoFrameTransform* t) { return t ? t->stream() : nullptr; }
 T360_API unsigned long long T360B200_kernelLaunchCount(void) { return t360::kernelLaunchCount(); }
+T360_API unsigned long long T360B200_stagedStoreLaunchCount(void) { return t360::stagedStoreLaunchCount(); }
 T360_API unsigned long long T360B200_planDeviceBytes(VideoFrameTransform* t, int planIndex) { return t ? t->planBytes(planIndex) : 0; }
 T360_API int T360B200_planTileCounts(VideoFrameTransform* t, int planIndex, int counts[4]) {
   return t && counts ? t->tileCounts(planIndex, counts) : 0;
diff --git a/transform360_b200/handler.py b/transform360_b200/handler.py
--- a/transform360_b200/handler.py
+++ b/transform360_b200/handler.py
@@ -234,6 +234,7 @@
     L.T360B200_stream.restype = vp
     L.T360B200_stream.argtypes = [vp]
     L.T360B200_kernelLaunchCount.restype = C.c_ulonglong
+    L.T360B200_stagedStoreLaunchCount.restype = C.c_ulonglong
     L.T360B200_planDeviceBytes.restype = C.c_ulonglong
     L.T360B200_planDeviceBytes.argtypes = [vp, ci]
     L.T360B200_planTileCounts.restype = ci
@@ -257,7 +258,8 @@
     "T360B200_transformFrameOrientedAsync", "T360B200_orientedSamples", "T360B200_transformFramePoseAsync", "T360B200_poseSamples",
     "T360B200_lensMap", "T360B200_transformFrameLensAsync", "T360B200_lensBlendMaps", "T360B200_transformFrameLensBlendAsync",
     "T360B200_rectilinearMap", "T360B200_transformFrameRectilinearAsync", "T360B200_cameraMap", "T360B200_transformFrameCameraAsync",
-    "T360B200_setPinHostPlanes", "T360B200_debugTrace", "T360B200_debugTraceRead", "T360B200_synchronize", "T360B200_stream", "T360B200_kernelLaunchCount", "T360B200_planDeviceBytes",
+    "T360B200_setPinHostPlanes", "T360B200_debugTrace", "T360B200_debugTraceRead", "T360B200_synchronize", "T360B200_stream", "T360B200_kernelLaunchCount",
+    "T360B200_stagedStoreLaunchCount", "T360B200_planDeviceBytes",
     "T360B200_planTileCounts", "T360B200_deviceCount", "T360B200_version",
 ]
 
@@ -601,5 +603,9 @@
     return int(load().T360B200_kernelLaunchCount())
 
 
+def staged_store_launch_count() -> int:
+    return int(load().T360B200_stagedStoreLaunchCount())
+
+
 def device_count() -> int:
     return int(load().T360B200_deviceCount())
```

Measured after the change: 765,500, median of 6. No clear change (+0.6%).
